# Lewis-Stuart-11/3DGS-to-PC

Measured on NVIDIA H100. Metric: Mpoints/sec (sample+colour) at 3M Gaussians/200 cams, 1/2/4/8 H100 vs CPU ref, higher is better.
Workload: dtype f32

## Files before the change

### 3dgs-to-pc_b200/csrc/colour_common.cuh

```cuda
#pragma once
#include "common.cuh"

#define QT_FLAG_DROPPED 1
#define QT_FLAG_BIG 2

#define NODE_NONE 0
#define NODE_EMPTY 1
#define NODE_SPLIT 2
#define NODE_LEAF 3

#define G2PC_RANGE_MAX_LEVEL 8
#define G2PC_RANGE_EMPTY 0x00000001u
__host__ __device__ __forceinline__ uint32_t g2pc_pack_range(int xlo, int xhi, int ylo, int yhi) {
    return (uint32_t)xlo | ((uint32_t)xhi << 8) | ((uint32_t)ylo << 16) | ((uint32_t)yhi << 24);
}
__host__ __device__ __forceinline__ void g2pc_unpack_range(uint32_t r, int& xlo, int& xhi, int& ylo, int& yhi) {
    xlo = (int)(r & 255u); xhi = (int)((r >> 8) & 255u); ylo = (int)((r >> 16) & 255u); yhi = (int)(r >> 24);
}

__device__ __forceinline__ bool g2pc_frame_skipped(const uint32_t* fail, int frame) {
    return (uint32_t)(frame + 1) >= *fail;
}

__device__ __forceinline__ bool g2pc_report_skipped_frame(const uint32_t* fail, int frame, int32_t* header) {
    if (!g2pc_frame_skipped(fail, frame)) return false;
    if (threadIdx.x == 0) { header[G2PC_HDR_POISON] = (int32_t)*fail; header[G2PC_HDR_FRAME] = frame; }
    return true;
}

__device__ __forceinline__ void g2pc_write_frame_header(int32_t* header, uint32_t* fail, int frame, int num_leaves,
                                                        long long inst_total, int total_pix, int need_deeper,
                                                        int leaf_over, int cap_over) {
    header[G2PC_HDR_NUM_LEAVES] = num_leaves;
    header[G2PC_HDR_TOTAL_INST] = (int32_t)(inst_total & 0xFFFFFFFFll);
    header[G2PC_HDR_TOTAL_INST_HI] = (int32_t)(inst_total >> 32);
    header[G2PC_HDR_TOTAL_PIX] = total_pix;
    header[G2PC_HDR_NEED_DEEPER] = need_deeper;
    header[G2PC_HDR_LEAF_OVERFLOW] = leaf_over;
    header[G2PC_HDR_CAP_OVERFLOW] = cap_over;
    header[G2PC_HDR_FRAME] = frame;
    if (need_deeper | leaf_over | cap_over) atomicMin(fail, (uint32_t)(frame + 1));
    const uint32_t f = *(volatile uint32_t*)fail;
    header[G2PC_HDR_POISON] = f == 0xFFFFFFFFu ? 0 : (int32_t)f;
}

template <int NT, int CAP, typename K, typename KeyF>
__device__ __forceinline__ void g2pc_launch_order(K* s_sort, int nl, KeyF key, K index_mask, int32_t* leaf_order) {
    if (nl > CAP) {
        for (int i = threadIdx.x; i < nl; i += NT) leaf_order[i] = i;
        return;
    }
    int m = 1;
    while (m < nl) m <<= 1;
    for (int i = threadIdx.x; i < m; i += NT) s_sort[i] = i < nl ? key(i) : ~(K)0;
    __syncthreads();
    for (int k = 2; k <= m; k <<= 1) {
        for (int j = k >> 1; j > 0; j >>= 1) {
            for (int i = threadIdx.x; i < m; i += NT) {
                const int ixj = i ^ j;
                if (ixj > i) {
                    const K a = s_sort[i], b = s_sort[ixj];
                    const bool up = (i & k) == 0;
                    if ((a > b) == up) { s_sort[i] = b; s_sort[ixj] = a; }
                }
            }
            __syncthreads();
        }
    }
    for (int i = threadIdx.x; i < nl; i += NT) leaf_order[i] = (int)(s_sort[i] & index_mask);
}

__device__ __forceinline__ float ex2_approx(float x) {
    float r;
    asm("ex2.approx.ftz.f32 %0, %1;" : "=f"(r) : "f"(x));
    return r;
}

__device__ __forceinline__ uint32_t smem_u32(const void* p) { return (uint32_t)__cvta_generic_to_shared(p); }

__device__ __forceinline__ void mbar_init(unsigned long long* bar, int count) {
    asm volatile("mbarrier.init.shared::cta.b64 [%0], %1;" ::"r"(smem_u32(bar)), "r"(count) : "memory");
}
__device__ __forceinline__ void mbar_wait(unsigned long long* bar, uint32_t parity) {
    asm volatile(
        "{\n"
        ".reg .pred p;\n"
        "WAIT_%=:\n"
        "mbarrier.try_wait.parity.shared::cta.b64 p, [%0], %1;\n"
        "@p bra DONE_%=;\n"
        "bra WAIT_%=;\n"
        "DONE_%=:\n"
        "}\n" ::"r"(smem_u32(bar)), "r"(parity) : "memory");
}
__device__ __forceinline__ void tma_load_1d(void* dst, const void* src, uint32_t bytes, unsigned long long* bar) {
    asm volatile("fence.proxy.async.shared::cta;" ::: "memory");
    asm volatile("mbarrier.arrive.expect_tx.shared::cta.b64 _, [%0], %1;" ::"r"(smem_u32(bar)), "r"(bytes) : "memory");
    asm volatile("cp.async.bulk.shared::cluster.global.mbarrier::complete_tx::bytes [%0], [%1], %2, [%3];" ::"r"(
                     smem_u32(dst)), "l"(src), "r"(bytes), "r"(smem_u32(bar)) : "memory");
}
__device__ __forceinline__ void cp_async16(void* dst, const void* src) {
    asm volatile("cp.async.cg.shared.global [%0], [%1], 16;" ::"r"(smem_u32(dst)), "l"(src) : "memory");
}
__device__ __forceinline__ void cp_async_commit() { asm volatile("cp.async.commit_group;" ::: "memory"); }
template <int N>
__device__ __forceinline__ void cp_async_wait() { asm volatile("cp.async.wait_group %0;" ::"n"(N) : "memory"); }

__device__ __forceinline__ void id_ring_init(unsigned long long* bar) {
    mbar_init(&bar[0], 1); mbar_init(&bar[1], 1); mbar_init(&bar[2], 1);
    asm volatile("fence.mbarrier_init.release.cluster;" ::: "memory");
}
template <int CH>
__device__ __forceinline__ void id_ring_issue(uint32_t (*ids)[CH], unsigned long long* bar, const uint32_t* list,
                                              int cnt, int c) {
    const int nl = min(CH, cnt - c * CH);
    tma_load_1d(&ids[c % 3][0], list + (int64_t)c * CH, (uint32_t)(((nl + 3) & ~3) * 4), &bar[c % 3]);
}
__device__ __forceinline__ void id_ring_wait(unsigned long long* bar, uint32_t& phase_bits, int c) {
    const int s = c % 3;
    mbar_wait(&bar[s], (phase_bits >> s) & 1u);
    phase_bits ^= 1u << s;
}

__device__ __forceinline__ int next_work_item(int32_t* counter, int* s_item) {
    if (threadIdx.x == 0) *s_item = atomicAdd(counter, 1);
    __syncthreads();
    const int item = *s_item;
    __syncthreads();
    return item;
}

template <typename Kernel>
int g2pc_resident_ctas(Kernel kernel, int threads, size_t smem, int fallback_per_sm) {
    int dev = 0, sms = 132, per_sm = fallback_per_sm;
    cudaGetDevice(&dev);
    cudaDeviceGetAttribute(&sms, cudaDevAttrMultiProcessorCount, dev);
    if (cudaOccupancyMaxActiveBlocksPerMultiprocessor(&per_sm, kernel, threads, smem) != cudaSuccess || per_sm < 1)
        per_sm = fallback_per_sm;
    return sms * per_sm;
}

template <typename Coef>
__device__ __forceinline__ float sh_channel(Coef s, int deg, float x, float y, float z) {
    const float C0 = 0.28209479177387814f, C1 = 0.4886025119029199f;
    const float C2[5] = {1.0925484305920792f, -1.0925484305920792f, 0.31539156525252005f, -1.0925484305920792f,
                         0.5462742152960396f};
    const float C3[7] = {-0.5900435899266435f, 2.890611442640554f, -0.4570457994644658f, 0.3731763325901154f,
                         -0.4570457994644658f, 1.445305721320277f, -0.5900435899266435f};
    const float xx = x * x, yy = y * y, zz = z * z, xy = x * y, yz = y * z, xz = x * z;
    float r = C0 * s(0);
    if (deg > 0) {
        r = r - C1 * y * s(1) + C1 * z * s(2) - C1 * x * s(3);
        if (deg > 1) {
            r = r + C2[0] * xy * s(4) + C2[1] * yz * s(5) + C2[2] * (2.0f * zz - xx - yy) * s(6) + C2[3] * xz * s(7) +
                C2[4] * (xx - yy) * s(8);
            if (deg > 2) {
                r = r + C3[0] * y * (3.0f * xx - yy) * s(9) + C3[1] * xy * z * s(10) +
                    C3[2] * y * (4.0f * zz - xx - yy) * s(11) + C3[3] * z * (2.0f * zz - 3.0f * xx - 3.0f * yy) * s(12) +
                    C3[4] * x * (4.0f * zz - xx - yy) * s(13) + C3[5] * z * (xx - yy) * s(14) +
                    C3[6] * x * (xx - 3.0f * yy) * s(15);
            }
        }
    }
    return fmaxf(r + 0.5f, 0.0f);
}

__host__ __device__ __forceinline__ int off2d(int l) { return ((1 << (2 * l)) - 1) / 3; }

struct QtMeta {
    int32_t num_levels;
    int32_t max_gaussians_per_tile;
    int32_t width, height;
};

struct QtTables {
    const int32_t* xs; const int32_t* xe; const int32_t* xf;
    const int32_t* ys; const int32_t* ye; const int32_t* yf;
};

inline QtTables make_tables(const int32_t* tables, int n1) {
    QtTables t;
    t.xs = tables; t.xe = tables + n1; t.xf = tables + 2 * n1;
    t.ys = tables + 3 * n1; t.ye = tables + 4 * n1; t.yf = tables + 5 * n1;
    return t;
}

__device__ __forceinline__ QtTables load_tables(const QtTables g, int n1, int32_t* smem) {
    for (int i = threadIdx.x; i < n1; i += blockDim.x) {
        smem[i] = g.xs[i];
        smem[n1 + i] = g.xe[i];
        smem[2 * n1 + i] = g.xf[i];
        smem[3 * n1 + i] = g.ys[i];
        smem[4 * n1 + i] = g.ye[i];
        smem[5 * n1 + i] = g.yf[i];
    }
    __syncthreads();
    QtTables s;
    s.xs = smem; s.xe = smem + n1; s.xf = smem + 2 * n1;
    s.ys = smem + 3 * n1; s.ye = smem + 4 * n1; s.yf = smem + 5 * n1;
    return s;
}

__device__ __forceinline__ void axis_range(const int32_t* __restrict__ s, const int32_t* __restrict__ e, int level,
                                           float rmin, float rmax, float inv_step, int& lo, int& hi) {
    const int n = 1 << level;
    if (!(rmax > rmin)) { lo = 1; hi = 0; return; }
    int a = min(n - 1, max(0, (int)(rmin * inv_step)));
    while (a < n && !((float)e[a] > rmin)) ++a;
    while (a > 0 && (float)e[a - 1] > rmin) --a;
    lo = a;
    a = min(n - 1, max(0, (int)(rmax * inv_step)));
    while (a >= 0 && !((float)s[a] < rmax)) --a;
    while (a + 1 < n && (float)s[a + 1] < rmax) ++a;
    hi = a;
}

__device__ __forceinline__ void axis_range_from(const int32_t* __restrict__ s, const int32_t* __restrict__ e, int level,
                                                float rmin, float rmax, int lo_guess, int hi_guess, int& lo, int& hi) {
    const int n = 1 << level;
    if (!(rmax > rmin)) { lo = 1; hi = 0; return; }
    int a = min(n - 1, max(0, lo_guess));
    while (a < n && !((float)e[a] > rmin)) ++a;
    while (a > 0 && (float)e[a - 1] > rmin) --a;
    lo = a;
    a = min(n - 1, max(0, hi_guess));
    while (a >= 0 && !((float)s[a] < rmax)) --a;
    while (a + 1 < n && (float)s[a + 1] < rmax) ++a;
    hi = a;
}

__device__ __forceinline__ bool axis_member(const int32_t* __restrict__ s, const int32_t* __restrict__ e,
                                            const int32_t* __restrict__ f, int i) {
    return !(f[i] & QT_FLAG_DROPPED) && e[i] > s[i];
}

constexpr int WARP_SMALL_AREA = 12;
template <typename F>
__device__ __forceinline__ void warp_for_each_node(uint32_t range, uint32_t payload, F f) {
    const int lane = threadIdx.x & 31;
    int xlo, xhi, ylo, yhi;
    g2pc_unpack_range(range, xlo, xhi, ylo, yhi);
    const int area = (xlo > xhi || ylo > yhi) ? 0 : (xhi - xlo + 1) * (yhi - ylo + 1);
    if (area > 0 && area <= WARP_SMALL_AREA)
        for (int iy = ylo; iy <= yhi; ++iy)
            for (int ix = xlo; ix <= xhi; ++ix) f(ix, iy, lane, payload);
    unsigned big = __ballot_sync(0xffffffffu, area > WARP_SMALL_AREA);
    while (big) {
        const int b = __ffs(big) - 1;
        big &= big - 1u;
        const uint32_t br = __shfl_sync(0xffffffffu, range, b);
        const uint32_t bp = __shfl_sync(0xffffffffu, payload, b);
        int bx, bxh, by, byh;
        g2pc_unpack_range(br, bx, bxh, by, byh);
        const int bw = bxh - bx + 1, bh = byh - by + 1;
        const int sh = bw <= 1 ? 0 : 32 - __clz(bw - 1);
        if (sh >= 5) {
            for (int ry = 0; ry < bh; ++ry)
                for (int rx = lane; rx < bw; rx += 32) f(bx + rx, by + ry, b, bp);
        } else {
            const int rx = lane & ((1 << sh) - 1);
            if (rx < bw)
                for (int ry = lane >> sh; ry < bh; ry += 32 >> sh) f(bx + rx, by + ry, b, bp);
        }
    }
}

__device__ __forceinline__ void gaussian_rect(float mx, float my, float radius, int W, int H, float& x0, float& x1,
                                              float& y0, float& y1) {
    const float wm = (float)W - 1.0f, hm = (float)H - 1.0f;
    x0 = fminf(fmaxf(mx - radius, 0.0f), wm);
    x1 = fminf(fmaxf(mx + radius, 0.0f), wm);
    y0 = fminf(fmaxf(my - radius, 0.0f), hm);
    y1 = fminf(fmaxf(my + radius, 0.0f), hm);
}
```

### 3dgs-to-pc_b200/csrc/core.cu

```cuda
#include <stdarg.h>
#include "common.cuh"

static thread_local char g_err[512] = "";

void g2pc_set_error(const char* fmt, ...) {
    va_list ap;
    va_start(ap, fmt);
    vsnprintf(g_err, sizeof(g_err), fmt, ap);
    va_end(ap);
}

extern "C" int g2pc_version(void) { return 110; }
extern "C" const char* g2pc_last_error(void) { return g_err; }
```

### 3dgs-to-pc_b200/csrc/s4_tree.cu

```cuda
#include <cub/cub.cuh>
#include "colour_common.cuh"

namespace {

constexpr int TB = 1024;
constexpr int SORT_CAP = 4096;

struct TreeParams {
    QtMeta meta;
    QtTables tab;
    int32_t n1;
    uint32_t* node_cnt;
    uint8_t* node_state;
    int32_t* node_leaf;
    g2pc_leaf_t* leaves;
    int32_t* leaf_order;
    int32_t max_leaves;
    int64_t inst_capacity, pix_capacity, matrix_capacity;
    int32_t ms_chunks;
    int32_t frame;
    int32_t* header;
    uint32_t* fail;
    int32_t* work_counters;
    int32_t nodes_2d;
};

__device__ __forceinline__ void deinterleave(int key, int level, int& ix, int& iy) {
    ix = 0; iy = 0;
    for (int b = 0; b < level; ++b) {
        iy |= ((key >> (2 * b)) & 1) << b;
        ix |= ((key >> (2 * b + 1)) & 1) << b;
    }
}

__global__ void __launch_bounds__(TB) tree_kernel(const TreeParams p) {
    __shared__ int s_warp[33];
    __shared__ int s_flags[2];
    __shared__ unsigned long long s_sort[SORT_CAP];
    if (g2pc_report_skipped_frame(p.fail, p.frame, p.header)) return;
    const int L = p.meta.num_levels;
    if (threadIdx.x == 0) { s_flags[0] = 0; s_flags[1] = 0; }
    __syncthreads();
    int leaf_base = 0;
    long long inst_total = 0;
    for (int l = 0; l < L; ++l) {
        const int nn = 1 << (2 * l);
        const int o1 = (1 << l) - 1, o2 = off2d(l);
        for (int k0 = 0; k0 < nn; k0 += TB) {
            const int key = k0 + threadIdx.x;
            int is_leaf = 0, node = -1, ix = 0, iy = 0;
            uint32_t cnt = 0;
            if (key < nn) {
                deinterleave(key, l, ix, iy);
                node = o2 + (iy << l) + ix;
                bool exists = (l == 0);
                if (l > 0) {
                    const int pnode = off2d(l - 1) + ((iy >> 1) << (l - 1)) + (ix >> 1);
                    exists = p.node_state[pnode] == NODE_SPLIT;
                }
                uint8_t st = NODE_NONE;
                int32_t nl = -1;
                if (exists) {
                    const int fx = p.tab.xf[o1 + ix], fy = p.tab.yf[o1 + iy];
                    if (!((fx | fy) & QT_FLAG_DROPPED)) {
                        cnt = p.node_cnt[node];
                        const bool big = ((fx | fy) & QT_FLAG_BIG) != 0;
                        if (cnt == 0) st = NODE_EMPTY;
                        else if (big || cnt > (uint32_t)p.meta.max_gaussians_per_tile) {
                            st = NODE_SPLIT;
                            nl = -2;
                            if (l == L - 1) { st = NODE_NONE; nl = -1; s_flags[0] = 1; }
                        } else {
                            st = NODE_LEAF;
                            is_leaf = 1;
                        }
                    }
                }
                p.node_state[node] = st;
                p.node_leaf[node] = nl;
            }
            int tot;
            const int pre = block_scan_1024(is_leaf, s_warp, tot);
            if (is_leaf) {
                const int li = leaf_base + pre;
                if (li < p.max_leaves) {
                    g2pc_leaf_t lf;
                    lf.r0 = p.tab.ys[o1 + iy];
                    lf.c0 = p.tab.xs[o1 + ix];
                    lf.w = p.tab.xe[o1 + ix] - lf.c0 + 1;
                    lf.h = p.tab.ye[o1 + iy] - lf.r0 + 1;
                    lf.inst_begin = 0;
                    lf.inst_count = (int32_t)cnt;
                    lf.pix_offset = 0;
                    lf.node = node;
                    p.leaves[li] = lf;
                    p.node_leaf[node] = li;
                } else {
                    s_flags[1] = 1;
                }
            }
            leaf_base += tot;
        }
        __syncthreads();
    }
    const int nl = leaf_base < p.max_leaves ? leaf_base : p.max_leaves;
    int pix_base = 0;
    for (int k0 = 0; k0 < nl; k0 += TB) {
        const int i = k0 + threadIdx.x;
        int c = 0, a = 0;
        if (i < nl) { c = (p.leaves[i].inst_count + 3) & ~3; a = p.leaves[i].w * p.leaves[i].h; }
        int tc, ta;
        const int pc = block_scan_1024(c, s_warp, tc);
        const int pa = block_scan_1024(a, s_warp, ta);
        if (i < nl) {
            p.leaves[i].inst_begin = (int32_t)(inst_total + pc);
            p.leaves[i].pix_offset = pix_base + pa;
        }
        inst_total += tc;
        pix_base += ta;
    }
    __syncthreads();
    g2pc_launch_order<TB, SORT_CAP>(s_sort, nl, [&](int i) {
        unsigned long long w = (unsigned long long)p.leaves[i].inst_count *
                               (unsigned long long)(p.leaves[i].w * p.leaves[i].h);
        w = w < (1ull << 44) - 1ull ? w : (1ull << 44) - 1ull;
        return (((1ull << 44) - 1ull - w) << 16) | (unsigned long long)i;
    }, 0xFFFFull, p.leaf_order);
    for (int k = threadIdx.x; k < p.nodes_2d; k += TB) p.node_cnt[k] = 0u;
    if (threadIdx.x < G2PC_WORK_COUNTERS) p.work_counters[threadIdx.x] = 0;
    if (threadIdx.x == 0) {
        const int cap_over = (inst_total > p.inst_capacity || (long long)pix_base > p.pix_capacity ||
                              (long long)p.ms_chunks * (long long)nl > p.matrix_capacity || inst_total > 0x7FFFFFFFll)
                                 ? 1 : 0;
        g2pc_write_frame_header(p.header, p.fail, p.frame, leaf_base, inst_total, pix_base, s_flags[0], s_flags[1],
                                cap_over);
    }
}

struct MsParams {
    const unsigned long long* val_sorted;
    int64_t n;
    const float4* proj;
    int32_t width, height;
    float inv_width, inv_height;
    QtMeta meta;
    QtTables tab;
    int32_t n1;
    uint32_t level_mask;
    int32_t base_level;
    const int32_t* node_leaf;
    const int32_t* header;
    const uint32_t* fail;
    int32_t frame;
    const g2pc_leaf_t* leaves;
    uint32_t* matrix;
    uint32_t* inst_gid;
    int32_t leaf_cap;
    int32_t base_clean;
    uint32_t clean_mask;
    int32_t grid_w;
    int32_t steps;
};

template <typename F>
__device__ __forceinline__ void for_each_leaf(const MsParams& p, const QtTables& T, const int32_t* __restrict__ s_leaf,
                                              uint32_t range, uint32_t gid, F f) {
    if (p.grid_w > 0) {
        warp_for_each_node(range, gid, [&](int ix, int iy, int owner, uint32_t og) { f(iy * p.grid_w + ix, owner, og); });
        return;
    }
    const int lb = p.base_level;
    const int o1 = (1 << lb) - 1;
    unsigned deeper = 0;
    if (p.base_clean) {
        warp_for_each_node(range, gid, [&](int ix, int iy, int owner, uint32_t og) {
            const int32_t v = s_leaf[(iy << lb) + ix];
            if (v >= 0) f(v, owner, og);
            else if (v == -2) deeper |= 1u << owner;
        });
    } else {
        warp_for_each_node(range, gid, [&](int ix, int iy, int owner, uint32_t og) {
            if (!axis_member(T.ys + o1, T.ye + o1, T.yf + o1, iy) || !axis_member(T.xs + o1, T.xe + o1, T.xf + o1, ix)) return;
            const int32_t v = s_leaf[(iy << lb) + ix];
            if (v >= 0) f(v, owner, og);
            else if (v == -2) deeper |= 1u << owner;
        });
    }
    if (p.meta.num_levels <= lb + 1) return;
    int xlo, xhi, ylo, yhi;
    g2pc_unpack_range(range, xlo, xhi, ylo, yhi);
#pragma unroll
    for (int o = 16; o > 0; o >>= 1) deeper |= __shfl_xor_sync(0xffffffffu, deeper, o);
    const int lane = threadIdx.x & 31;
    bool mine = (deeper >> lane) & 1u;
    if (!mine && xlo <= xhi) {
        const int ex = max(xlo - 1, 0), ey = max(ylo - 1, 0);
        for (int iy = ey; iy <= yhi; ++iy)
            for (int ix = ex; ix <= xhi; ++ix)
                if ((iy < ylo || ix < xlo) && s_leaf[(iy << lb) + ix] == -2) mine = true;
    }
    if (!__any_sync(0xffffffffu, mine)) return;
    float x0 = 0.f, x1 = 0.f, y0 = 0.f, y1 = 0.f;
    if (mine) {
        const float4 q0 = __ldg(p.proj + 3 * (int64_t)gid);
        const float4 q2 = __ldg(p.proj + 3 * (int64_t)gid + 2);
        gaussian_rect(q0.x, q0.y, q2.z, p.width, p.height, x0, x1, y0, y1);
    }
    const float isx0 = p.inv_width, isy0 = p.inv_height;
    for (int l = lb + 1; l < p.meta.num_levels; ++l) {
        if (!((p.level_mask >> l) & 1u)) continue;
        const int ol = (1 << l) - 1;
        int axlo = 1, axhi = 0, aylo = 1, ayhi = 0;
        if (mine) {
            axis_range(T.xs + ol, T.xe + ol, l, x0, x1, isx0 * (float)(1 << l), axlo, axhi);
            if (axlo <= axhi) axis_range(T.ys + ol, T.ye + ol, l, y0, y1, isy0 * (float)(1 << l), aylo, ayhi);
        }
        const bool some = axlo <= axhi && aylo <= ayhi;
        const int32_t* nl = p.node_leaf + off2d(l);
        if (((p.clean_mask >> l) & 1u) && l <= G2PC_RANGE_MAX_LEVEL) {
            const uint32_t rl = some ? g2pc_pack_range(axlo, axhi, aylo, ayhi) : (uint32_t)G2PC_RANGE_EMPTY;
            warp_for_each_node(rl, gid, [&](int ix, int iy, int owner, uint32_t og) {
                const int32_t v = __ldg(nl + (iy << l) + ix);
                if (v >= 0) f(v, owner, og);
            });
            continue;
        }
        if (!some) continue;
        for (int iy = aylo; iy <= ayhi; ++iy) {
            if (!axis_member(T.ys + ol, T.ye + ol, T.yf + ol, iy)) continue;
            for (int ix = axlo; ix <= axhi; ++ix) {
                if (!axis_member(T.xs + ol, T.xe + ol, T.xf + ol, ix)) continue;
                const int32_t v = __ldg(nl + (iy << l) + ix);
                if (v >= 0) f(v, lane, gid);
            }
        }
    }
}

__device__ __forceinline__ unsigned long long ms_entry(const MsParams& p, int64_t k) {
    return k < p.n ? p.val_sorted[k] : (unsigned long long)G2PC_RANGE_EMPTY << 32;
}

__device__ __forceinline__ int32_t* ms_load_common(const MsParams& p, int32_t* smem, QtTables& T) {
    if (p.grid_w > 0) { T = p.tab; return smem; }
    if (p.base_clean && p.meta.num_levels <= p.base_level + 1) {
        T = p.tab;
        __syncthreads();
    } else {
        T = load_tables(p.tab, p.n1, smem);
    }
    int32_t* s_leaf = smem + 6 * p.n1;
    const int nb = 1 << (2 * p.base_level);
    const int32_t* src = p.node_leaf + off2d(p.base_level);
    for (int i = threadIdx.x; i < nb; i += blockDim.x) s_leaf[i] = src[i];
    return s_leaf;
}

template <int C>
__global__ void __launch_bounds__(C, 1024 / C) ms_count_kernel(const MsParams p) {
    extern __shared__ int32_t smem_ms[];
    if (g2pc_frame_skipped(p.fail, p.frame)) return;
    const int nl = p.header[G2PC_HDR_NUM_LEAVES];
    QtTables T;
    int32_t* s_leaf = ms_load_common(p, smem_ms, T);
    uint32_t* s_hist = reinterpret_cast<uint32_t*>(s_leaf + (p.grid_w > 0 ? 0 : (1 << (2 * p.base_level))));
    for (int i = threadIdx.x; i < nl; i += C) s_hist[i] = 0u;
    __syncthreads();
    const int64_t k0 = (int64_t)blockIdx.x * p.steps * C;
    for (int s = 0; s < p.steps; ++s) {
        const int64_t b = k0 + (int64_t)s * C;
        if (b >= p.n) break;
        const unsigned long long v = ms_entry(p, b + threadIdx.x);
        for_each_leaf(p, T, s_leaf, (uint32_t)(v >> 32), (uint32_t)v,
                      [&](int leaf, int, uint32_t) { atomicAdd(s_hist + leaf, 1u); });
    }
    __syncthreads();
    uint32_t* row = p.matrix + (int64_t)blockIdx.x * nl;
    for (int i = threadIdx.x; i < nl; i += C) row[i] = s_hist[i];
}

constexpr int SCAN_BATCH = 8;
__global__ void __launch_bounds__(1024) ms_scan_kernel(const MsParams p, int32_t rows) {
    __shared__ uint32_t s_sum[32][33];
    if (g2pc_frame_skipped(p.fail, p.frame)) return;
    const int nl = p.header[G2PC_HDR_NUM_LEAVES];
    if (blockIdx.x * 32 >= nl) return;
    const int tx = threadIdx.x & 31, ty = threadIdx.x >> 5;
    const int leaf = blockIdx.x * 32 + tx;
    const int band = (rows + 31) / 32;
    const int r0 = min(rows, ty * band), r1 = min(rows, r0 + band);
    uint32_t* col = p.matrix + leaf;
    uint32_t sum = 0;
    if (leaf < nl) {
#pragma unroll 8
        for (int r = r0; r < r1; ++r) sum += col[(int64_t)r * nl];
    }
    s_sum[ty][tx] = sum;
    __syncthreads();
    if (leaf >= nl) return;
    uint32_t run = (uint32_t)p.leaves[leaf].inst_begin;
    for (int s = 0; s < ty; ++s) run += s_sum[s][tx];
    for (int r = r0; r < r1; r += SCAN_BATCH) {
        uint32_t c[SCAN_BATCH];
#pragma unroll
        for (int q = 0; q < SCAN_BATCH; ++q) c[q] = r + q < r1 ? col[(int64_t)(r + q) * nl] : 0u;
#pragma unroll
        for (int q = 0; q < SCAN_BATCH; ++q) {
            if (r + q < r1) col[(int64_t)(r + q) * nl] = run;
            run += c[q];
        }
    }
}

template <int C>
__global__ void __launch_bounds__(C, 768 / C) ms_scatter_kernel(const MsParams p) {
    extern __shared__ int32_t smem_ms[];
    if (g2pc_frame_skipped(p.fail, p.frame)) return;
    const int nl = p.header[G2PC_HDR_NUM_LEAVES];
    constexpr int WORDS = C / 32;
    QtTables T;
    int32_t* s_leaf = ms_load_common(p, smem_ms, T);
    uint32_t* s_row = reinterpret_cast<uint32_t*>(s_leaf + (p.grid_w > 0 ? 0 : (1 << (2 * p.base_level))));
    uint32_t* s_bits = s_row + p.leaf_cap;
    {
        const uint32_t* grow = p.matrix + (int64_t)blockIdx.x * nl;
        for (int i = threadIdx.x; i < nl; i += C) s_row[i] = grow[i];
        if (((reinterpret_cast<uintptr_t>(s_bits) & 15) == 0) && ((nl & 3) == 0)) {
            uint4* b4 = reinterpret_cast<uint4*>(s_bits);
            for (int i = threadIdx.x; i < WORDS * nl / 4; i += C) b4[i] = make_uint4(0u, 0u, 0u, 0u);
        } else {
            for (int i = threadIdx.x; i < WORDS * nl; i += C) s_bits[i] = 0u;
        }
    }
    __syncthreads();
    const int w = threadIdx.x >> 5;
    uint32_t* mybits = s_bits + w * nl;
    const int64_t k0 = (int64_t)blockIdx.x * p.steps * C;
    unsigned long long v = ms_entry(p, k0 + threadIdx.x);
    for (int s = 0; s < p.steps; ++s) {
        const int64_t b = k0 + (int64_t)s * C;
        if (b >= p.n) break;
        const bool more = s + 1 < p.steps && b + C < p.n;
        const uint32_t range = (uint32_t)(v >> 32), gid = (uint32_t)v;
        for_each_leaf(p, T, s_leaf, range, gid, [&](int leaf, int owner, uint32_t) { atomicOr(mybits + leaf, 1u << owner); });
        __syncthreads();
        const unsigned long long vn = more ? ms_entry(p, b + C + threadIdx.x) : 0ull;
        for_each_leaf(p, T, s_leaf, range, gid, [&](int leaf, int owner, uint32_t og) {
            uint32_t pos = s_row[leaf] + (uint32_t)__popc(mybits[leaf] & ((1u << owner) - 1u));
            for (int w2 = 0; w2 < w; ++w2) pos += (uint32_t)__popc(s_bits[w2 * nl + leaf]);
            p.inst_gid[pos] = og;
        });
        if (!more) break;
        __syncthreads();
        for (int i = threadIdx.x; i < nl; i += C) {
            uint32_t cnt = 0;
#pragma unroll
            for (int w2 = 0; w2 < WORDS; ++w2) {
                cnt += (uint32_t)__popc(s_bits[w2 * nl + i]);
                s_bits[w2 * nl + i] = 0u;
            }
            s_row[i] += cnt;
        }
        __syncthreads();
        v = vn;
    }
}

size_t align256(size_t x) { return (x + 255) & ~(size_t)255; }

constexpr int64_t MS_TARGET_CTAS = 4096;
constexpr int64_t MS_MAX_STEPS = 32;
int32_t ms_steps(int64_t n, int C) {
    const int64_t s = n / ((int64_t)C * MS_TARGET_CTAS);
    return (int32_t)(s < 1 ? 1 : (s > MS_MAX_STEPS ? MS_MAX_STEPS : s));
}

int32_t ms_chunks(int64_t n, int C) {
    const int64_t e = (int64_t)C * ms_steps(n, C);
    return (int32_t)((n + e - 1) / e);
}

template <int C>
int launch_multisplit(const MsParams& p, int32_t chunks, cudaStream_t st) {
    const size_t common = p.grid_w > 0 ? 0 : ((size_t)6 * p.n1 + ((size_t)1 << (2 * p.base_level))) * sizeof(int32_t);
    const size_t smem_count = common + (size_t)p.leaf_cap * sizeof(uint32_t);
    const size_t smem_scatter = common + (size_t)(C / 32 + 1) * p.leaf_cap * sizeof(uint32_t);
    if (smem_scatter > 200 * 1024 || smem_count > 200 * 1024) {
        g2pc_set_error("g2pc_multisplit: shared memory budget exceeded");
        return G2PC_ERR_INVALID;
    }
    if (smem_count > 48 * 1024)
        G2PC_CUDA(cudaFuncSetAttribute(ms_count_kernel<C>, cudaFuncAttributeMaxDynamicSharedMemorySize, (int)smem_count));
    if (smem_scatter > 48 * 1024)
        G2PC_CUDA(cudaFuncSetAttribute(ms_scatter_kernel<C>, cudaFuncAttributeMaxDynamicSharedMemorySize, (int)smem_scatter));
    ms_count_kernel<C><<<(unsigned)chunks, C, smem_count, st>>>(p);
    G2PC_CHECK_LAUNCH();
    ms_scan_kernel<<<(unsigned)((p.leaf_cap + 31) / 32), 1024, 0, st>>>(p, chunks);
    G2PC_CHECK_LAUNCH();
    ms_scatter_kernel<C><<<(unsigned)chunks, C, smem_scatter, st>>>(p);
    G2PC_CHECK_LAUNCH();
    return G2PC_OK;
}

int run_multisplit(MsParams p, int C, cudaStream_t st) {
    p.steps = ms_steps(p.n, C);
    const int32_t chunks = ms_chunks(p.n, C);
    if (C == 256) return launch_multisplit<256>(p, chunks, st);
    if (C == 128) return launch_multisplit<128>(p, chunks, st);
    return launch_multisplit<64>(p, chunks, st);
}

}

extern "C" int g2pc_build_tree(const int32_t* tables, int32_t num_levels, int32_t max_gaussians_per_tile,
                               uint32_t* node_cnt, uint8_t* node_state, int32_t* node_leaf, g2pc_leaf_t* leaves,
                               int32_t* leaf_order, int32_t max_leaves, int64_t inst_capacity, int64_t pix_capacity,
                               int64_t matrix_capacity, int32_t ms_chunks, int32_t frame, int32_t* header,
                               uint32_t* fail, int32_t* work_counters, void* stream) {
    G2PC_CHECK_ARG(tables && node_cnt && node_state && node_leaf && leaves && leaf_order && header && fail &&
                       work_counters, "null pointer");
    G2PC_CHECK_ARG(num_levels >= 1 && num_levels <= G2PC_MAX_LEVELS && max_leaves >= 1, "bad sizes");
    G2PC_CHECK_ARG(frame >= 0 && ms_chunks >= 0, "bad frame / chunk count");
    TreeParams p;
    p.meta.num_levels = num_levels; p.meta.max_gaussians_per_tile = max_gaussians_per_tile;
    p.meta.width = 0; p.meta.height = 0;
    p.n1 = (1 << num_levels) - 1;
    p.tab = make_tables(tables, p.n1);
    p.node_cnt = node_cnt; p.node_state = node_state; p.node_leaf = node_leaf; p.leaves = leaves;
    p.leaf_order = leaf_order; p.max_leaves = max_leaves;
    p.inst_capacity = inst_capacity; p.pix_capacity = pix_capacity; p.matrix_capacity = matrix_capacity;
    p.ms_chunks = ms_chunks; p.frame = frame; p.header = header; p.fail = fail; p.work_counters = work_counters;
    p.nodes_2d = off2d(num_levels);
    tree_kernel<<<1, TB, 0, (cudaStream_t)stream>>>(p);
    G2PC_CHECK_LAUNCH();
    return G2PC_OK;
}

extern "C" int64_t g2pc_depth_sort_workspace_bytes(int64_t n) {
    size_t sort_b = 0;
    cub::DeviceRadixSort::SortPairs(nullptr, sort_b, (const uint32_t*)nullptr, (uint32_t*)nullptr,
                                    (const unsigned long long*)nullptr, (unsigned long long*)nullptr, n);
    return (int64_t)(align256((size_t)n * 4) + align256(sort_b));
}

extern "C" int g2pc_depth_sort(const uint32_t* depth_key, const uint64_t* val, int64_t n, uint64_t* val_sorted,
                               void* workspace, int64_t workspace_bytes, void* stream) {
    G2PC_CHECK_ARG(n >= 0, "n < 0");
    if (n == 0) return G2PC_OK;
    G2PC_CHECK_ARG(depth_key && val && val_sorted && workspace, "null pointer");
    G2PC_CHECK_ARG(workspace_bytes >= g2pc_depth_sort_workspace_bytes(n), "workspace too small");
    char* ws = (char*)workspace;
    uint32_t* keys_out = (uint32_t*)ws;
    void* tmp = ws + align256((size_t)n * 4);
    size_t b = (size_t)workspace_bytes - align256((size_t)n * 4);
    G2PC_CUDA(cub::DeviceRadixSort::SortPairs(tmp, b, depth_key, keys_out, (const unsigned long long*)val,
                                              (unsigned long long*)val_sorted, n, 0, 32, (cudaStream_t)stream));
    return G2PC_OK;
}

extern "C" int32_t g2pc_multisplit_chunk(int32_t leaf_cap) {
    const int64_t n = leaf_cap;
    if (n * 36 <= 74 * 1024) return 256;
    if (n * 20 <= 74 * 1024) return 128;
    if (n * 12 <= 110 * 1024) return 64;
    if (n * 20 <= 200 * 1024) return 128;
    if (n * 12 <= 200 * 1024) return 64;
    return 0;
}

extern "C" int32_t g2pc_multisplit_rows(int64_t n, int32_t leaf_cap) {
    const int C = g2pc_multisplit_chunk(leaf_cap);
    if (C <= 0) return 0;
    return ms_chunks(n, C);
}

extern "C" int g2pc_multisplit(const uint64_t* val_sorted, int64_t n, const void* proj, int32_t width, int32_t height,
                               const int32_t* tables, int32_t num_levels, uint32_t level_mask, uint32_t clean_mask,
                               const int32_t* node_leaf,
                               const g2pc_leaf_t* leaves, const int32_t* header, const uint32_t* fail, int32_t frame,
                               int32_t leaf_cap, uint32_t* matrix, uint32_t* inst_gid, void* stream) {
    G2PC_CHECK_ARG(n >= 0, "n < 0");
    if (n == 0) return G2PC_OK;
    G2PC_CHECK_ARG(val_sorted && proj && tables && node_leaf && leaves && header && fail && matrix && inst_gid,
                   "null pointer");
    G2PC_CHECK_ARG(num_levels >= 1 && num_levels <= G2PC_MAX_LEVELS && level_mask != 0u, "bad levels");
    const int C = g2pc_multisplit_chunk(leaf_cap);
    G2PC_CHECK_ARG(C > 0, "too many leaves for the multisplit");
    MsParams p;
    p.val_sorted = (const unsigned long long*)val_sorted; p.n = n; p.proj = (const float4*)proj;
    p.width = width; p.height = height;
    p.inv_width = 1.0f / (float)width; p.inv_height = 1.0f / (float)height;
    p.meta.num_levels = num_levels; p.meta.max_gaussians_per_tile = 0; p.meta.width = width; p.meta.height = height;
    p.n1 = (1 << num_levels) - 1;
    p.tab = make_tables(tables, p.n1);
    p.level_mask = level_mask; p.base_level = __builtin_ctz(level_mask);
    G2PC_CHECK_ARG(p.base_level <= G2PC_RANGE_MAX_LEVEL, "first leaf-candidate level too deep");
    p.node_leaf = node_leaf; p.header = header; p.fail = fail; p.frame = frame; p.leaves = leaves; p.matrix = matrix;
    p.inst_gid = inst_gid;
    p.leaf_cap = leaf_cap; p.grid_w = 0;
    p.base_clean = (int32_t)((clean_mask >> p.base_level) & 1u);
    p.clean_mask = clean_mask;
    return run_multisplit(p, C, (cudaStream_t)stream);
}

extern "C" int g2pc_multisplit_grid(const uint64_t* val_sorted, int64_t n, int32_t grid_w, int32_t grid_h,
                                    const g2pc_leaf_t* leaves, const int32_t* header, const uint32_t* fail,
                                    int32_t frame, int32_t leaf_cap, uint32_t* matrix, uint32_t* inst_gid, void* stream) {
    G2PC_CHECK_ARG(n >= 0, "n < 0");
    if (n == 0) return G2PC_OK;
    G2PC_CHECK_ARG(val_sorted && leaves && header && fail && matrix && inst_gid, "null pointer");
    G2PC_CHECK_ARG(grid_w >= 1 && grid_h >= 1 && grid_w <= 256 && grid_h <= 256 && leaf_cap >= grid_w * grid_h,
                   "bad tile grid / leaf_cap");
    const int C = g2pc_multisplit_chunk(leaf_cap);
    G2PC_CHECK_ARG(C > 0, "too many tiles for the multisplit");
    MsParams p{};
    p.val_sorted = (const unsigned long long*)val_sorted; p.n = n;
    p.meta.num_levels = 1;
    p.level_mask = 1u;
    p.header = header; p.fail = fail; p.frame = frame; p.leaves = leaves; p.matrix = matrix;
    p.inst_gid = inst_gid;
    p.leaf_cap = leaf_cap; p.grid_w = grid_w; p.base_clean = 1; p.clean_mask = 1u;
    return run_multisplit(p, C, (cudaStream_t)stream);
}
```

### 3dgs-to-pc_b200/g2pc/capi.py

```python
import contextlib
import ctypes
import os

import torch

HERE = os.path.dirname(os.path.abspath(__file__))
LIB_PATH = os.path.join(HERE, "libg2pc.so")

F32, F64 = 0, 1
CULL_EPS_NORM, CULL_EXPLICIT = 0, 1
ST_OVERFLOW, ST_CHOLFAIL, ST_CHOLREG, ST_WORDS = 0, 1, 2, 4

_c_void_p = ctypes.c_void_p
_i32, _i64, _u32, _u64, _f32 = ctypes.c_int32, ctypes.c_int64, ctypes.c_uint32, ctypes.c_uint64, ctypes.c_float

SIGNATURES = {
    "g2pc_version": ([], ctypes.c_int),
    "g2pc_last_error": ([], ctypes.c_char_p),
    "g2pc_cov_build": ([_c_void_p, _c_void_p, ctypes.c_int, _f32, _i64, _c_void_p, _c_void_p], ctypes.c_int),
    "g2pc_normals": ([_c_void_p, _c_void_p, ctypes.c_int, _i64, _c_void_p, _c_void_p], ctypes.c_int),
    "g2pc_eigvals_sym3": ([_c_void_p, _i64, _c_void_p, _c_void_p], ctypes.c_int),
    "g2pc_sample_count": ([_c_void_p, _c_void_p, _c_void_p, ctypes.c_int, _c_void_p, _c_void_p, _c_void_p, _i64, _i64,
                           _c_void_p, _i32, _i32, _i32, _f32, _i32, _u64, _u32, _c_void_p, _c_void_p, _c_void_p,
                           _c_void_p, _c_void_p], ctypes.c_int),
    "g2pc_sample_emit_chunk_points": ([], ctypes.c_int),
    "g2pc_sample_emit": ([_c_void_p, _c_void_p, _i64, _c_void_p, _c_void_p, _c_void_p, _i32, _u64, _u32, _c_void_p,
                          _c_void_p, _c_void_p, ctypes.c_int, _i64, _c_void_p], ctypes.c_int),
    "g2pc_dump_eps": ([_c_void_p, _i64, _i32, _i32, _u64, _u32, _c_void_p, _c_void_p], ctypes.c_int),
    "g2pc_cull_workspace_bytes": ([_i64], ctypes.c_int64),
    "g2pc_cull_select": ([_c_void_p, _f32, _c_void_p, _f32, _c_void_p, _c_void_p, _c_void_p, _c_void_p, _c_void_p,
                          _c_void_p, _i64, _i64, _i64, _c_void_p, _c_void_p, _c_void_p, _i64, _c_void_p], ctypes.c_int),
    "g2pc_gather_rows": ([_c_void_p, _i64, _i32, _c_void_p, _c_void_p, _c_void_p, _c_void_p], ctypes.c_int),
    "g2pc_ppg_workspace_bytes": ([_i64], ctypes.c_int64),
    "g2pc_knn_workspace_bytes": ([_i64], ctypes.c_int64),
    "g2pc_knn_mean_dist": ([_c_void_p, _i64, _i32, _c_void_p, _c_void_p, _c_void_p, _i64, _c_void_p], ctypes.c_int),
    "g2pc_knn_ids": ([_c_void_p, _i64, _i32, _c_void_p, _c_void_p, _c_void_p, _c_void_p, _i64, _c_void_p], ctypes.c_int),
    "g2pc_sor_workspace_bytes": ([_i64], ctypes.c_int64),
    "g2pc_sor_mask": ([_c_void_p, _i64, ctypes.c_double, _c_void_p, _c_void_p, _c_void_p, _i64, _c_void_p], ctypes.c_int),
    "g2pc_mesh_splat_workspace_bytes": ([_i64], ctypes.c_int64),
    "g2pc_mesh_splat": ([_c_void_p, _c_void_p, ctypes.c_int, _i64, _i32, _c_void_p, _c_void_p, _c_void_p, _c_void_p,
                         _c_void_p, _i64, _c_void_p], ctypes.c_int),
    "g2pc_mesh_solve_workspace_bytes": ([_i32], ctypes.c_int64),
    "g2pc_mesh_vcycle": ([_c_void_p, _c_void_p, _i32, _c_void_p, _i32, _c_void_p, _c_void_p, _i64, _c_void_p],
                         ctypes.c_int),
    "g2pc_mesh_iso_workspace_bytes": ([], ctypes.c_int64),
    "g2pc_mesh_iso": ([_c_void_p, _c_void_p, _i64, _c_void_p, _i32, _c_void_p, _c_void_p, _c_void_p, _i64, _c_void_p],
                      ctypes.c_int),
    "g2pc_mesh_extract_workspace_bytes": ([_i32], ctypes.c_int64),
    "g2pc_mesh_extract_count": ([_c_void_p, _i32, _c_void_p, _c_void_p, _c_void_p, _i64, _c_void_p], ctypes.c_int),
    "g2pc_mesh_extract_emit": ([_c_void_p, _i32, _c_void_p, _c_void_p, _c_void_p, _i64, _c_void_p, _i64, _c_void_p,
                                _c_void_p, _c_void_p, _c_void_p, _c_void_p], ctypes.c_int),
    "g2pc_mesh_gather_workspace_bytes": ([_i64], ctypes.c_int64),
    "g2pc_mesh_gather": ([_c_void_p, _c_void_p, _c_void_p, _i64, _c_void_p, _i32, _c_void_p, _c_void_p, _i64, _c_void_p,
                          _i64, _c_void_p, _c_void_p, _c_void_p, _i64, _c_void_p], ctypes.c_int),
    "g2pc_mesh_trim_workspace_bytes": ([_i64, _i64], ctypes.c_int64),
    "g2pc_mesh_trim": ([_c_void_p, _c_void_p, _c_void_p, _i64, _c_void_p, _i64, _c_void_p, _c_void_p, _c_void_p,
                        _c_void_p, _c_void_p, _c_void_p, _c_void_p, _c_void_p, _i64, _c_void_p], ctypes.c_int),
    "g2pc_mesh_smooth_workspace_bytes": ([_i64, _i64], ctypes.c_int64),
    "g2pc_mesh_smooth": ([_c_void_p, _i64, _c_void_p, _i64, _i32, _c_void_p, _i64, _c_void_p], ctypes.c_int),
    "g2pc_mesh_normals_workspace_bytes": ([_i64, _i64], ctypes.c_int64),
    "g2pc_mesh_normals": ([_c_void_p, _i64, _c_void_p, _i64, _c_void_p, _c_void_p, _c_void_p, _i64, _c_void_p],
                          ctypes.c_int),
    "g2pc_mesh_band_bricks_workspace_bytes": ([_i32], ctypes.c_int64),
    "g2pc_mesh_band_bricks": ([_c_void_p, _c_void_p, _i64, _c_void_p, _i32, _c_void_p, _c_void_p, _c_void_p, _c_void_p,
                               _c_void_p, _i64, _c_void_p], ctypes.c_int),
    "g2pc_mesh_band_list": ([_c_void_p, _i32, _c_void_p, _c_void_p], ctypes.c_int),
    "g2pc_mesh_band_splat": ([_c_void_p, _c_void_p, ctypes.c_int, _c_void_p, _i64, _c_void_p, _i32, _c_void_p, _i64,
                              _c_void_p, _c_void_p, _c_void_p], ctypes.c_int),
    "g2pc_mesh_band_ghosts": ([_c_void_p, _c_void_p, _i32, _c_void_p, _c_void_p, _i64, _c_void_p, _c_void_p, _c_void_p,
                               _c_void_p, _c_void_p, _c_void_p], ctypes.c_int),
    "g2pc_mesh_band_cg_workspace_bytes": ([_i64], ctypes.c_int64),
    "g2pc_mesh_band_cg_start": ([_c_void_p, _i32, _c_void_p, _c_void_p, _i64, _c_void_p, _c_void_p, _c_void_p, _i64,
                                 _c_void_p], ctypes.c_int),
    "g2pc_mesh_band_cg_step": ([_c_void_p, _i32, _c_void_p, _c_void_p, _i64, _c_void_p, _i32, _c_void_p, _c_void_p,
                                _i64, _c_void_p], ctypes.c_int),
    "g2pc_mesh_band_iso_workspace_bytes": ([], ctypes.c_int64),
    "g2pc_mesh_band_iso": ([_c_void_p, _c_void_p, _i64, _c_void_p, _i32, _c_void_p, _c_void_p, _c_void_p, _c_void_p,
                            _i64, _c_void_p], ctypes.c_int),
    "g2pc_mesh_band_extract_workspace_bytes": ([_i64], ctypes.c_int64),
    "g2pc_mesh_band_extract_count": ([_c_void_p, _i32, _c_void_p, _c_void_p, _i64, _c_void_p, _c_void_p, _c_void_p,
                                      _i64, _c_void_p], ctypes.c_int),
    "g2pc_mesh_band_extract_emit": ([_c_void_p, _i32, _c_void_p, _c_void_p, _i64, _c_void_p, _c_void_p, _c_void_p, _i64,
                                     _c_void_p, _i64, _c_void_p, _c_void_p, _c_void_p, _c_void_p, _c_void_p],
                                    ctypes.c_int),
    "g2pc_mesh_band_gather_workspace_bytes": ([_i64], ctypes.c_int64),
    "g2pc_mesh_band_gather": ([_c_void_p, _c_void_p, _c_void_p, _i64, _c_void_p, _i32, _c_void_p, _c_void_p, _i64,
                               _c_void_p, _c_void_p, _c_void_p, _i64, _c_void_p], ctypes.c_int),
    "g2pc_mesh_decimate_prepare_workspace_bytes": ([_i64, _i64], ctypes.c_int64),
    "g2pc_mesh_decimate_prepare": ([_c_void_p, _i64, _c_void_p, _i64, _c_void_p, _c_void_p, _c_void_p, _i64, _c_void_p],
                                   ctypes.c_int),
    "g2pc_mesh_decimate_round_workspace_bytes": ([_i64, _i64], ctypes.c_int64),
    "g2pc_mesh_decimate_select": ([_c_void_p, _i64, _c_void_p, _i64, _c_void_p, _c_void_p, _c_void_p, _c_void_p, _i64,
                                   _c_void_p], ctypes.c_int),
    "g2pc_mesh_decimate_apply": ([_c_void_p, _i64, _c_void_p, _i64, _c_void_p, _c_void_p, _c_void_p, _c_void_p,
                                  _c_void_p, _i64, _i64, _c_void_p, _c_void_p, _c_void_p, _c_void_p, _c_void_p, _i64,
                                  _c_void_p], ctypes.c_int),
    "g2pc_mesh_decimate_finish_workspace_bytes": ([_i64], ctypes.c_int64),
    "g2pc_mesh_decimate_finish": ([_c_void_p, _i64, _c_void_p, _i64, _c_void_p, _c_void_p, _c_void_p, _c_void_p,
                                   _c_void_p, _c_void_p, _c_void_p, _c_void_p, _c_void_p, _c_void_p, _i64, _c_void_p],
                                  ctypes.c_int),
    "g2pc_tsdf_frame_workspace_bytes": ([_i64], ctypes.c_int64),
    "g2pc_tsdf_frame": ([_c_void_p, _i64, _i32, _c_void_p, _c_void_p, _i64, _c_void_p], ctypes.c_int),
    "g2pc_tsdf_integrate": ([_c_void_p, _i32, ctypes.c_double, _c_void_p, _c_void_p, _c_void_p, _c_void_p, _i32, _i32,
                             _c_void_p, _c_void_p, _c_void_p, _i32, _c_void_p, _c_void_p, _c_void_p, _c_void_p],
                            ctypes.c_int),
    "g2pc_tsdf_compact_workspace_bytes": ([_i64, _i64], ctypes.c_int64),
    "g2pc_tsdf_gather_compact": ([_c_void_p, _c_void_p, _i32, _c_void_p, _c_void_p, _c_void_p, _i64, _c_void_p, _i64,
                                  _c_void_p, _c_void_p, _c_void_p, _c_void_p, _c_void_p, _c_void_p, _c_void_p,
                                  _c_void_p, _c_void_p, _i64, _c_void_p], ctypes.c_int),
    "g2pc_orient_prepare_workspace_bytes": ([_i64], ctypes.c_int64),
    "g2pc_orient_prepare": ([_c_void_p, _c_void_p, ctypes.c_int, _i64, _c_void_p, _c_void_p, _c_void_p, _c_void_p,
                             _c_void_p, _i64, _c_void_p], ctypes.c_int),
    "g2pc_orient_edges_workspace_bytes": ([_i64, _i32], ctypes.c_int64),
    "g2pc_orient_edges": ([_c_void_p, _i64, _i32, _c_void_p, _c_void_p, _c_void_p, _c_void_p, _c_void_p, _c_void_p,
                           _i64, _c_void_p], ctypes.c_int),
    "g2pc_orient_round_workspace_bytes": ([_i64, _i64], ctypes.c_int64),
    "g2pc_orient_round": ([_c_void_p, _c_void_p, _c_void_p, _i64, _i64, _i32, _i64, _c_void_p, _c_void_p, _c_void_p,
                           _c_void_p, _c_void_p, _i64, _c_void_p], ctypes.c_int),
    "g2pc_orient_finish_workspace_bytes": ([_i64], ctypes.c_int64),
    "g2pc_orient_finish": ([_c_void_p, _c_void_p, _c_void_p, _i64, _c_void_p, ctypes.c_int, _i64, _c_void_p, _c_void_p,
                            _c_void_p, _c_void_p, _c_void_p, _c_void_p, _c_void_p, _i64, _c_void_p], ctypes.c_int),
    "g2pc_face_cameras": ([_c_void_p, _c_void_p, ctypes.c_int, _c_void_p, _i64, _c_void_p, _i64, _c_void_p, _i64,
                           _c_void_p, _c_void_p, _c_void_p], ctypes.c_int),
    "g2pc_points_per_gaussian": ([_c_void_p, _c_void_p, _i64, ctypes.c_double, _c_void_p, _c_void_p, _c_void_p, _i64,
                                  _c_void_p], ctypes.c_int),
    "g2pc_pack_geometry": ([_c_void_p, _c_void_p, _c_void_p, _i64, _c_void_p, _c_void_p], ctypes.c_int),
    "g2pc_preprocess": ([_c_void_p, _c_void_p, _c_void_p, _i32, _i32, _i64, _c_void_p, _c_void_p, _c_void_p, _i32, _u32,
                         _u32, _c_void_p, _c_void_p, _c_void_p, _c_void_p, _c_void_p], ctypes.c_int),
    "g2pc_preprocess_cameras": ([_c_void_p, _c_void_p, _c_void_p, _i32, _i32, _i64, _c_void_p, _i32, _c_void_p,
                                 _c_void_p, _i32, _u32, _u32, _c_void_p, _c_void_p, _c_void_p, _c_void_p, _c_void_p],
                                ctypes.c_int),
    "g2pc_depth_sort_workspace_bytes": ([_i64], ctypes.c_int64),
    "g2pc_depth_sort": ([_c_void_p, _c_void_p, _i64, _c_void_p, _c_void_p, _i64, _c_void_p], ctypes.c_int),
    "g2pc_build_tree": ([_c_void_p, _i32, _i32, _c_void_p, _c_void_p, _c_void_p, _c_void_p, _c_void_p, _i32, _i64, _i64,
                         _i64, _i32, _i32, _c_void_p, _c_void_p, _c_void_p, _c_void_p], ctypes.c_int),
    "g2pc_multisplit_chunk": ([_i32], ctypes.c_int32),
    "g2pc_multisplit_rows": ([_i64, _i32], ctypes.c_int32),
    "g2pc_multisplit": ([_c_void_p, _i64, _c_void_p, _i32, _i32, _c_void_p, _i32, _u32, _u32, _c_void_p, _c_void_p,
                         _c_void_p, _c_void_p, _i32, _i32, _c_void_p, _c_void_p, _c_void_p], ctypes.c_int),
    "g2pc_blend": ([_c_void_p, _c_void_p, _c_void_p, _c_void_p, _i32, _i32, _i32, _c_void_p, _c_void_p, _c_void_p,
                    _c_void_p, _c_void_p, _c_void_p, _i32, _i32, _f32, _f32, _c_void_p, _c_void_p, _c_void_p],
                   ctypes.c_int),
    "g2pc_blend_set_compact": ([ctypes.c_int], None),
    "g2pc_blend_set_cull": ([ctypes.c_int], None),
    "g2pc_accumulate": ([_c_void_p, _c_void_p, _i64, _c_void_p, _c_void_p, _c_void_p, _i32, _c_void_p], ctypes.c_int),
    "g2pc_tiles_preprocess": ([_c_void_p, _c_void_p, _c_void_p, _i32, _i32, _i32, _i64, _c_void_p, _c_void_p, _c_void_p,
                               _c_void_p, _c_void_p, _c_void_p, _c_void_p], ctypes.c_int),
    "g2pc_tiles_build": ([_c_void_p, _i32, _i32, _c_void_p, _c_void_p, _i32, _i64, _i64, _i32, _i32, _c_void_p,
                          _c_void_p, _c_void_p, _c_void_p], ctypes.c_int),
    "g2pc_multisplit_grid": ([_c_void_p, _i64, _i32, _i32, _c_void_p, _c_void_p, _c_void_p, _i32, _i32, _c_void_p,
                              _c_void_p, _c_void_p], ctypes.c_int),
    "g2pc_tiles_blend": ([_c_void_p, _c_void_p, _c_void_p, _c_void_p, _i32, _c_void_p, _c_void_p, _c_void_p, _c_void_p,
                          _c_void_p, _c_void_p, _c_void_p, _c_void_p, _i32, _i32, _c_void_p, _c_void_p, _c_void_p,
                          _c_void_p], ctypes.c_int),
    "g2pc_tiles_blend_fusion": ([_c_void_p, _c_void_p, _c_void_p, _c_void_p, _i32, _c_void_p, _c_void_p, _c_void_p,
                                 _c_void_p, _c_void_p, _c_void_p, _c_void_p, _c_void_p, _i32, _i32, _c_void_p, _c_void_p,
                                 _c_void_p, _c_void_p, _c_void_p, _c_void_p], ctypes.c_int),
    "g2pc_tiles_accumulate": ([_c_void_p, _c_void_p, _c_void_p, _i32, _i32, _i64, _c_void_p, _c_void_p, _c_void_p,
                               _c_void_p, _c_void_p, _i32, _c_void_p, _c_void_p, _c_void_p, _c_void_p], ctypes.c_int),
    "g2pc_fill_u32": ([_c_void_p, _u32, _i64, _c_void_p], ctypes.c_int),
    "g2pc_compose_image": ([_c_void_p, _c_void_p, _i32, _i32, _f32, _c_void_p, _c_void_p], ctypes.c_int),
}


class Raster(ctypes.Structure):
    _fields_ = [("viewmatrix", _f32 * 16), ("projmatrix", _f32 * 16), ("campos", _f32 * 3), ("tan_fovx", _f32),
                ("tan_fovy", _f32), ("width", _i32), ("height", _i32)]


class Camera(ctypes.Structure):
    _fields_ = [("view", _f32 * 16), ("proj", _f32 * 16), ("campos", _f32 * 3), ("tan_fovx", _f32),
                ("tan_fovy", _f32), ("focal_x", _f32), ("focal_y", _f32), ("width", _i32), ("height", _i32)]


(HDR_NUM_LEAVES, HDR_TOTAL_INST, HDR_TOTAL_PIX, HDR_NEED_DEEPER, HDR_LEAF_OVERFLOW, HDR_CAP_OVERFLOW, HDR_POISON,
 HDR_FRAME, HDR_TOTAL_INST_HI) = range(9)
HDR_WORDS = 16
WORK_COUNTERS = 4
STAT_WARP_GAUSSIANS, STAT_WORDS = 0, 4
LEAF_WORDS = 8
PREPROCESS_MAX_CAMERAS = 8

_lib = None


class G2pcError(RuntimeError):
    pass


def load(path=None):
    global _lib
    if _lib is not None and path is None:
        return _lib
    path = path or LIB_PATH
    if not os.path.exists(path):
        raise G2pcError(
            f"{path} not found: build it with `python -m g2pc.build` (or __graft_entry__.build()). "
            "There is no CPU fallback for the g2pc kernels.")
    lib = ctypes.CDLL(path)
    for name, (argtypes, restype) in SIGNATURES.items():
        fn = getattr(lib, name)
        fn.argtypes = argtypes
        fn.restype = restype
    _lib = lib
    return lib


LAUNCHES = 0
TIMING = None
_OWN_KERNELS = {"g2pc_multisplit": 3, "g2pc_multisplit_grid": 3, "g2pc_depth_sort": 0, "g2pc_cull_select": 3,
                "g2pc_points_per_gaussian": 5, "g2pc_knn_mean_dist": 6, "g2pc_knn_ids": 6, "g2pc_sor_mask": 5, "g2pc_mesh_splat": 5,
                "g2pc_mesh_iso": 7, "g2pc_mesh_extract_count": 2, "g2pc_mesh_extract_emit": 2, "g2pc_mesh_gather": 3,
                "g2pc_mesh_trim": 6, "g2pc_mesh_normals": 3, "g2pc_mesh_band_bricks": 4, "g2pc_mesh_band_cg_start": 4,
                "g2pc_mesh_band_cg_step": 6,
                "g2pc_mesh_band_iso": 4, "g2pc_mesh_band_extract_count": 2, "g2pc_mesh_band_extract_emit": 2,
                "g2pc_mesh_band_gather": 2, "g2pc_mesh_decimate_prepare": 4, "g2pc_mesh_decimate_select": 8,
                "g2pc_mesh_decimate_apply": 5, "g2pc_mesh_decimate_finish": 4, "g2pc_orient_prepare": 2, "g2pc_orient_edges": 2,
                "g2pc_orient_round": 5, "g2pc_orient_finish": 3, "g2pc_tsdf_frame": 2, "g2pc_tsdf_gather_compact": 4}
_NOT_KERNELS = {"g2pc_version", "g2pc_last_error", "g2pc_sample_emit_chunk_points", "g2pc_multisplit_chunk",
                "g2pc_multisplit_rows", "g2pc_blend_set_compact", "g2pc_blend_set_cull"}


def call(name, *args):
    global LAUNCHES
    fn = getattr(load(), name)
    if TIMING is None or name in _NOT_KERNELS or name.endswith("_workspace_bytes"):
        status = fn(*args)
    else:
        with phase(TIMING, name):
            status = fn(*args)
    LAUNCHES += _OWN_KERNELS.get(name, 1)
    check(status, name)


@contextlib.contextmanager
def phase(timings, name):
    if timings is None:
        yield
        return
    a, b = torch.cuda.Event(enable_timing=True), torch.cuda.Event(enable_timing=True)
    a.record()
    yield
    b.record()
    timings.setdefault(name, []).append((a, b))


def check(status, what):
    if status != 0:
        msg = load().g2pc_last_error()
        raise G2pcError(f"{what} failed (status {status}): {msg.decode() if msg else ''}")


def ptr(t):
    if t is None:
        return None
    return t.data_ptr()


def workspace(nbytes, device):
    return torch.empty((max(int(nbytes), 256),), dtype=torch.uint8, device=device)


def stream_ptr(device=None):
    return torch.cuda.current_stream(device).cuda_stream


def dtype_code(t):
    if t.dtype == torch.float32:
        return F32
    if t.dtype == torch.float64:
        return F64
    raise G2pcError(f"unsupported dtype {t.dtype} (need float32 or float64)")


def require_cuda(*tensors):
    for t in tensors:
        if t is not None and not t.is_cuda:
            raise G2pcError("g2pc kernels need CUDA tensors; there is no CPU fallback "
                            f"(got a tensor on {t.device})")


def check_cloud(points, normals=None, colours=None, what=None):
    if what is not None and normals is None:
        raise G2pcError(f"{what} needs normals (the cloud has none)")
    if points is None:
        raise G2pcError(f"{what or 'the point-cloud kernels'} needs the points")
    require_cuda(points, normals, colours)
    if points.dim() != 2 or points.shape[1] != 3 or points.dtype != torch.float32:
        raise G2pcError(f"points must be (n, 3) float32, got {tuple(points.shape)} {points.dtype}")
    if normals is not None and (normals.shape != points.shape or normals.dtype not in (torch.float32, torch.float64)):
        raise G2pcError(f"normals must be (n, 3) float32 or float64 like the points, got {tuple(normals.shape)} "
                        f"{normals.dtype}")
    if colours is not None and colours.shape != points.shape:
        raise G2pcError(f"colours must be (n, 3) like the points, got {tuple(colours.shape)}")
    devices = [str(t.device) for t in (points, normals, colours) if t is not None]
    if len(set(devices)) > 1:
        raise G2pcError(f"the points, normals and colours are on different devices ({', '.join(devices)})")


def gather_rows(index, m, tensors):
    dev = index.device
    srcs = [t.contiguous() for t in tensors]
    dsts = [torch.empty((m,) + tuple(s.shape[1:]), dtype=s.dtype, device=dev) for s in srcs]
    if m > 0:
        k = len(srcs)
        call("g2pc_gather_rows", ptr(index), m, k, (ctypes.c_void_p * k)(*[s.data_ptr() for s in srcs]),
             (ctypes.c_void_p * k)(*[d.data_ptr() for d in dsts]),
             (ctypes.c_int32 * k)(*[s[0].numel() * s.element_size() for s in srcs]), stream_ptr(dev))
    return dsts
```

### 3dgs-to-pc_b200/g2pc/frames.py

```python
import torch

from . import capi, config


_HDR_POOLS = {}


def _resolution(camera):
    return int(camera.image_width), int(camera.image_height)


def total_instances(h):
    return h[capi.HDR_TOTAL_INST] + (h[capi.HDR_TOTAL_INST_HI] << 32)


class FrameQueue:

    def _init_frames(self, preprocess_cameras=1):
        self._frame = 0
        self._pending = []
        self._deferred = []
        self._batch = 0
        self.preprocess_cameras = preprocess_cameras
        self._hdr_pool = _HDR_POOLS.setdefault(str(self.device), [])
        self.replays = 0
        self.async_mode = False
        self.num_slots = max(1, int(config.FRAME_SLOTS))
        self._streams = [torch.cuda.Stream(device=self.device) for _ in range(self.num_slots)]
        self._fail = torch.full((1,), -1, dtype=torch.int32, device=self.device)
        self._prev_done = None
        dev, m = self.device, max(self._n, 1)
        nbytes = int(self.lib.g2pc_depth_sort_workspace_bytes(m))
        self._slots = [dict(proj=torch.empty((m, 12), dtype=torch.float32, device=dev),
                            depth_key=torch.empty((m,), dtype=torch.int32, device=dev),
                            val=torch.empty((m,), dtype=torch.int64, device=dev),
                            val_sorted=torch.empty((m,), dtype=torch.int64, device=dev),
                            depth_ws=torch.empty((max(nbytes, 1),), dtype=torch.uint8, device=dev),
                            hdr=torch.zeros((capi.HDR_WORDS,), dtype=torch.int32, device=dev),
                            work=torch.zeros((capi.WORK_COUNTERS,), dtype=torch.int32, device=dev),
                            inst_gid=None, matrix=None) for _ in range(self.num_slots)]
        self._pre_sets = [[sl] + [None] * (preprocess_cameras - 1) for sl in self._slots]
        self._set_free = [None] * self.num_slots
        self._pre_stream = torch.cuda.Stream(device=self.device) if preprocess_cameras > 1 else None
        self._cam_best = torch.zeros((m,), dtype=torch.int64, device=dev)
        self._stats = torch.zeros((capi.STAT_WORDS,), dtype=torch.int64, device=dev)
        self._inst_cap = max(8 * self._n, 1 << 16)
        self._tables = {}
        self._last_slot = 0
        self.last_stats = {}

    def _grow_lists(self, sl, leaf_cap, rows):
        need = self._inst_cap + 4 * leaf_cap + 64
        if sl["inst_gid"] is None or sl["inst_gid"].numel() < need:
            sl["inst_gid"] = torch.empty((need,), dtype=torch.int32, device=self.device)
        mneed = rows * leaf_cap
        if sl["matrix"] is None or sl["matrix"].numel() < mneed:
            sl["matrix"] = torch.empty((max(mneed, 1),), dtype=torch.int32, device=self.device)

    def _depth_sort(self, sl, stream, pre=None):
        pre = sl if pre is None else pre
        capi.call("g2pc_depth_sort", capi.ptr(pre["depth_key"]), capi.ptr(pre["val"]), self._n, capi.ptr(sl["val_sorted"]),
                  capi.ptr(sl["depth_ws"]), sl["depth_ws"].numel(), stream)

    def _grow_inst_cap(self, h):
        total = total_instances(h)
        if total > 0x7FFFFFFF:
            raise capi.G2pcError(f"{total} (Gaussian, tile) instances in one camera: more than 2^31 - 1")
        self._inst_cap = max(self._inst_cap, int(1.25 * total) + 1024)

    def _reset_counts(self):
        for t in self._tables.values():
            for ts in t["slots"]:
                ts["node_cnt"].zero_()
            for cnts in t.get("pre_cnt", []):
                for c in cnts:
                    c.zero_()

    def executed_pairs(self):
        self.flush()
        return int(self._stats[capi.STAT_WARP_GAUSSIANS].item()) * 128

    def get_gaussian_colours(self):
        self.flush()
        return self.gaussian_colours * 255

    def _pre_set(self, bset, j):
        sets = self._pre_sets[bset]
        if sets[j] is None:
            m = max(self._n, 1)
            sets[j] = dict(proj=torch.empty((m, 12), dtype=torch.float32, device=self.device),
                           depth_key=torch.empty((m,), dtype=torch.int32, device=self.device),
                           val=torch.empty((m,), dtype=torch.int64, device=self.device))
        return sets[j]

    def _enqueue_preprocess(self, cameras, bset):
        """Owners whose front half projects each camera itself (the CUDA back-end) have nothing to do here."""

    def _launch_batch(self, batch):
        bset = self._batch % self.num_slots
        self._batch += 1
        for j, (frame, camera, _) in enumerate(batch):
            self._ensure_buffers(camera, frame % self.num_slots)
            self._pre_set(bset, j)
        ready = torch.cuda.Event()
        ready.record(torch.cuda.current_stream(self.device))
        st0 = self._pre_stream if self._pre_stream is not None else self._streams[batch[0][0] % self.num_slots]
        st0.wait_event(ready)
        if self._set_free[bset] is not None:
            st0.wait_event(self._set_free[bset])
        with torch.cuda.stream(st0):
            self._enqueue_preprocess([camera for _, camera, _ in batch], bset)
        projected = torch.cuda.Event()
        projected.record(st0)
        for j, (frame, camera, camera_index) in enumerate(batch):
            slot = frame % self.num_slots
            st = self._streams[slot]
            if st is not st0:
                st.wait_event(projected)
            with torch.cuda.stream(st):
                dev_hdr = self._enqueue_front(camera, frame, slot, (bset, j))
                hdr = self._hdr_pool.pop() if self._hdr_pool else torch.zeros((capi.HDR_WORDS,), dtype=torch.int32).pin_memory()
                hdr.copy_(dev_hdr, non_blocking=True)
                if self._prev_done is not None:
                    st.wait_event(self._prev_done)
                self._enqueue_back(camera, frame, camera_index, slot)
                done = torch.cuda.Event()
                done.record(st)
            self._prev_done = done
            self._pending.append((frame, camera, camera_index, hdr, done))
        self._set_free[bset] = self._prev_done

    def _launch_frames(self, frames):
        batch = []
        for item in frames:
            if batch and (len(batch) == self.preprocess_cameras or _resolution(batch[0][1]) != _resolution(item[1])):
                self._launch_batch(batch)
                batch = []
            batch.append(item)
        if batch:
            self._launch_batch(batch)

    def _submit(self, camera, camera_index=None):
        frame = self._frame
        self._frame += 1
        camera_index = frame if camera_index is None else camera_index
        self._deferred.append((frame, camera, camera_index))
        if not self.async_mode:
            self.flush()
        else:
            if len(self._deferred) >= self.preprocess_cameras:
                self._launch_deferred()
            self._poll(block_if_more_than=8)

    def _launch_deferred(self):
        frames, self._deferred = self._deferred, []
        self._launch_frames(frames)

    def _poll(self, block_if_more_than=None):
        while self._pending:
            frame, camera, cidx, hdr, ev = self._pending[0]
            if not ev.query():
                if block_if_more_than is None or len(self._pending) <= block_if_more_than:
                    return
                ev.synchronize()
            h = hdr.tolist()
            if h[capi.HDR_POISON] and h[capi.HDR_POISON] - 1 <= frame:
                self._recover(h)
                continue
            self._confirm(h)
            self._hdr_pool.append(hdr)
            self._pending.pop(0)

    def flush(self):
        self._launch_deferred()
        while self._pending:
            self._pending[-1][4].synchronize()
            self._poll(block_if_more_than=0)
        if self._prev_done is not None:
            torch.cuda.current_stream(self.device).wait_event(self._prev_done)

    def _all_streams(self):
        return self._streams + ([self._pre_stream] if self._pre_stream is not None else [])

    def _recover(self, h):
        for st in self._all_streams():
            st.synchronize()
        failed = h[capi.HDR_POISON] - 1
        todo = [p for p in self._pending if p[0] >= failed]
        self._pending = [p for p in self._pending if p[0] < failed]
        self._fix(h)
        self._fail.fill_(-1)
        self._reset_counts()
        torch.cuda.current_stream(self.device).synchronize()
        self.replays += 1
        for (frame, camera, cidx, hdr, ev) in todo:
            self._hdr_pool.append(hdr)
        self._launch_frames([(frame, camera, cidx) for (frame, camera, cidx, hdr, ev) in todo])

    def __del__(self):
        try:
            for st in self._all_streams():
                st.synchronize()
        except Exception:
            pass
```

### 3dgs-to-pc_b200/g2pc/rasterizer.py

```python
import ctypes
import math
from typing import NamedTuple

import torch

from . import capi
from .frames import FrameQueue, total_instances

FLT_MAX_BITS = 0x7F7FFFFF
TILE = 16


class GaussianRasterizationSettings(NamedTuple):
    image_height: int
    image_width: int
    tanfovx: float
    tanfovy: float
    bg: torch.Tensor
    scale_modifier: float
    viewmatrix: torch.Tensor
    projmatrix: torch.Tensor
    sh_degree: int
    campos: torch.Tensor
    mask: torch.Tensor
    prefiltered: bool
    debug: bool
    antialiasing: bool


def _host_list(t, n):
    if isinstance(t, (list, tuple)):
        v = [float(x) for x in t]
    else:
        v = t.detach().to("cpu", torch.float32).reshape(-1).tolist()
    if len(v) != n:
        raise ValueError(f"expected {n} values, got {len(v)}")
    return v


def _raster_struct(rs):
    c = capi.Raster()
    V = getattr(rs, "_viewmatrix_host", None) or _host_list(rs.viewmatrix, 16)
    P = getattr(rs, "_projmatrix_host", None) or _host_list(rs.projmatrix, 16)
    pos = getattr(rs, "_campos_host", None) or _host_list(rs.campos, 3)
    for i in range(16):
        c.viewmatrix[i] = V[i]
        c.projmatrix[i] = P[i]
    for i in range(3):
        c.campos[i] = pos[i]
    c.tan_fovx, c.tan_fovy = float(rs.tanfovx), float(rs.tanfovy)
    c.width, c.height = int(rs.image_width), int(rs.image_height)
    return c


def _cov6_to_full(cov6):
    c = cov6.to(torch.float32)
    return torch.stack([c[:, 0], c[:, 1], c[:, 2], c[:, 1], c[:, 3], c[:, 4], c[:, 2], c[:, 4], c[:, 5]], 1).reshape(-1, 3, 3)


def _cov_from_scale_rot(scales, rotations, mod):
    q = rotations.to(torch.float32)
    r, x, y, z = q[:, 0], q[:, 1], q[:, 2], q[:, 3]
    R = torch.stack([1 - 2 * (y * y + z * z), 2 * (x * y - r * z), 2 * (x * z + r * y),
                     2 * (x * y + r * z), 1 - 2 * (x * x + z * z), 2 * (y * z - r * x),
                     2 * (x * z - r * y), 2 * (y * z + r * x), 1 - 2 * (x * x + y * y)], 1).reshape(-1, 3, 3)
    L = R * (mod * scales.to(torch.float32))[:, None, :]
    return L @ L.transpose(1, 2)


class GaussianRasterizer(FrameQueue):

    def __init__(self, means3D, means2D, opacities, shs=None, colors_precomp=None, scales=None, rotations=None,
                 cov3D_precomp=None, visible_gaussian_threshold=0.0, surface_distance_std=None,
                 calculate_surface_distance=False, sh_layout=0):
        if (shs is None and colors_precomp is None) or (shs is not None and colors_precomp is not None):
            raise Exception('Please provide excatly one of either SHs or precomputed colors!')
        if ((scales is None or rotations is None) and cov3D_precomp is None) or \
                ((scales is not None or rotations is not None) and cov3D_precomp is not None):
            raise Exception('Please provide exactly one of either scale/rotation pair or precomputed 3D covariance!')
        capi.require_cuda(means3D, opacities, shs, colors_precomp, scales, rotations, cov3D_precomp)
        self.lib = capi.load()
        self.means3D = means3D.to(torch.float32).contiguous()
        self.means2D = means2D
        self.opacities = opacities
        self.shs = shs if shs is not None else torch.Tensor([])
        self.colors_precomp = colors_precomp if colors_precomp is not None else torch.Tensor([])
        self.scales = scales if scales is not None else torch.Tensor([])
        self.rotations = rotations if rotations is not None else torch.Tensor([])
        self.cov3D_precomp = cov3D_precomp if cov3D_precomp is not None else torch.Tensor([])
        self.device = self.means3D.device
        dev = self.device
        n = self.means3D.shape[0]
        self._n = n

        self.gaussian_max_contribution = torch.zeros(n, device=dev, dtype=torch.float)
        self.gaussian_min_surface_distance = torch.full((n,), torch.finfo(torch.float).max, device=dev, dtype=torch.float)
        self.gaussian_total_contribution = torch.zeros(n, device=dev, dtype=torch.float)
        self.gaussian_colours = torch.zeros((n, 3), device=dev, dtype=torch.float)
        self.visible_gaussian_threshold = visible_gaussian_threshold
        self.surface_distance_std = surface_distance_std
        self.calculate_surface_distance = calculate_surface_distance
        self.first_frame = None

        self._scale_modifier = None
        self._geom = torch.empty((max(n, 1), 12), dtype=torch.float32, device=dev)
        self._packed = False
        self._colour_f32 = colors_precomp.to(torch.float32).contiguous() if colors_precomp is not None else None
        self._shs_f32 = None
        self._sh_layout = int(sh_layout)
        if shs is not None:
            self._shs_f32 = shs.to(torch.float32).contiguous()
            self._sh_stride = int(self._shs_f32.shape[2] if self._sh_layout == 0 else self._shs_f32.shape[1])
        self._init_frames()
        m = max(n, 1)
        for sl in self._slots:
            sl["radii"] = torch.zeros((m,), dtype=torch.int32, device=dev)
        self._cam_dist = None
        if calculate_surface_distance:
            self._cam_dist = torch.empty((m,), dtype=torch.int32, device=dev)
            capi.call("g2pc_fill_u32", capi.ptr(self._cam_dist), FLT_MAX_BITS, m, capi.stream_ptr(dev))

    def __call__(self, raster_settings, **kw):
        return self.forward(raster_settings, **kw)

    def _pack(self, scale_modifier):
        if self._packed and self._scale_modifier == scale_modifier:
            return
        if self.cov3D_precomp.numel():
            cov = _cov6_to_full(self.cov3D_precomp) if self.cov3D_precomp.dim() == 2 else self.cov3D_precomp.to(torch.float32)
        else:
            cov = _cov_from_scale_rot(self.scales, self.rotations, float(scale_modifier))
        op = self.opacities.to(torch.float32).reshape(-1).contiguous()
        capi.call("g2pc_pack_geometry", capi.ptr(self.means3D), capi.ptr(cov.contiguous()), capi.ptr(op), self._n,
                  capi.ptr(self._geom), capi.stream_ptr(self.device))
        self._packed, self._scale_modifier = True, scale_modifier

    def _res_tables(self, W, H):
        t = self._tables.get((W, H))
        if t is None:
            dev = self.device
            gx, gy = ((W + TILE - 1) // TILE + 1) // 2, ((H + TILE - 1) // TILE + 1) // 2
            ntiles = gx * gy
            chunk = int(self.lib.g2pc_multisplit_chunk(ntiles))
            if chunk <= 0:
                raise capi.G2pcError(f"{ntiles} tiles: image too large for the multisplit tables")
            t = dict(gx=gx, gy=gy, ntiles=ntiles, rows=int(self.lib.g2pc_multisplit_rows(self._n, ntiles)),
                     slots=[dict(node_cnt=torch.zeros((ntiles,), dtype=torch.int32, device=dev),
                                 leaves=torch.zeros((ntiles, capi.LEAF_WORDS), dtype=torch.int32, device=dev),
                                 leaf_order=torch.zeros((ntiles,), dtype=torch.int32, device=dev))
                            for _ in range(self.num_slots)],
                     colour=torch.zeros((3, H, W), dtype=torch.float32, device=dev),
                     depth=torch.zeros((1, H, W), dtype=torch.float32, device=dev),
                     invdepth=torch.zeros((1, H, W), dtype=torch.float32, device=dev))
            self._tables[(W, H)] = t
        return t

    def _mask_of(self, rs, W, H):
        mask = rs.mask
        if mask is None:
            return None
        if not mask.is_cuda:
            raise capi.G2pcError("mask must be a CUDA tensor")
        if mask.numel() != W * H:
            raise capi.G2pcError("mask must have image_height * image_width entries")
        return mask.to(torch.int32).contiguous()

    def _ensure_buffers(self, rs, slot):
        self._pack(float(rs.scale_modifier))
        t = self._res_tables(int(rs.image_width), int(rs.image_height))
        self._grow_lists(self._slots[slot], t["ntiles"], t["rows"])
        self._slots[slot]["mask"] = self._mask_of(rs, int(rs.image_width), int(rs.image_height))

    def _enqueue_front(self, rs, frame, slot, pre=None):
        st = capi.stream_ptr(self.device)
        W, H = int(rs.image_width), int(rs.image_height)
        n = self._n
        t = self._res_tables(W, H)
        sl, ts = self._slots[slot], t["slots"][slot]
        c = _raster_struct(rs)
        deg = int(rs.sh_degree) if self._shs_f32 is not None else 0
        capi.call("g2pc_tiles_preprocess", capi.ptr(self._geom), capi.ptr(self._colour_f32), capi.ptr(self._shs_f32),
                  self._sh_stride if self._shs_f32 is not None else 0, min(deg, 3), self._sh_layout, n, ctypes.byref(c),
                  capi.ptr(sl["proj"]), capi.ptr(ts["node_cnt"]), capi.ptr(sl["depth_key"]), capi.ptr(sl["val"]),
                  capi.ptr(sl["radii"]), st)
        self._depth_sort(sl, st)
        capi.call("g2pc_tiles_build", capi.ptr(ts["node_cnt"]), W, H, capi.ptr(ts["leaves"]), capi.ptr(ts["leaf_order"]),
                  t["ntiles"], self._inst_cap, sl["matrix"].numel(), t["rows"], frame, capi.ptr(sl["hdr"]),
                  capi.ptr(self._fail), capi.ptr(sl["work"]), st)
        capi.call("g2pc_multisplit_grid", capi.ptr(sl["val_sorted"]), n, t["gx"], t["gy"], capi.ptr(ts["leaves"]),
                  capi.ptr(sl["hdr"]), capi.ptr(self._fail), frame, t["ntiles"], capi.ptr(sl["matrix"]),
                  capi.ptr(sl["inst_gid"]), st)
        self._last, self._last_slot = t, slot
        return sl["hdr"]

    def _enqueue_back(self, rs, frame, camera_index, slot):
        st = capi.stream_ptr(self.device)
        W, H = int(rs.image_width), int(rs.image_height)
        n = self._n
        t = self._res_tables(W, H)
        sl, ts = self._slots[slot], t["slots"][slot]
        mask = sl.get("mask")
        if mask is not None:
            t["colour"].zero_(); t["depth"].zero_(); t["invdepth"].zero_()
        bg = (ctypes.c_float * 3)(*(getattr(rs, "_bg_host", None) or _host_list(rs.bg, 3)))
        capi.call("g2pc_tiles_blend", capi.ptr(ts["leaves"]), capi.ptr(ts["leaf_order"]), capi.ptr(sl["hdr"]),
                  capi.ptr(self._fail), frame, capi.ptr(sl["inst_gid"]), capi.ptr(sl["proj"]), capi.ptr(self._cam_best),
                  capi.ptr(self._cam_dist), capi.ptr(mask), capi.ptr(t["colour"]), capi.ptr(t["depth"]),
                  capi.ptr(t["invdepth"]), W, H, bg, capi.ptr(sl["work"]), capi.ptr(self._stats), st)
        pc = getattr(self, "_per_camera", None) or (None, None, None)
        capi.call("g2pc_tiles_accumulate", capi.ptr(self._cam_best), capi.ptr(self._cam_dist), capi.ptr(t["colour"]), W, H,
                  n, capi.ptr(self.gaussian_max_contribution), capi.ptr(self.gaussian_total_contribution),
                  capi.ptr(self.gaussian_colours), capi.ptr(self.gaussian_min_surface_distance),
                  capi.ptr(self.first_frame), int(camera_index), capi.ptr(pc[0]), capi.ptr(pc[1]), capi.ptr(pc[2]), st)

    def forward(self, raster_settings, camera_index=None):
        self._submit(raster_settings, camera_index)
        t, radii = self._last, self._slots[self._last_slot]["radii"]
        if self.async_mode:
            return t["colour"], radii, t["invdepth"], t["depth"]
        return t["colour"].clone(), radii.clone(), t["invdepth"].clone(), t["depth"].clone()

    def _confirm(self, h):
        self.last_stats = dict(num_tiles=h[capi.HDR_NUM_LEAVES], frame=h[capi.HDR_FRAME],
                               total_instances=total_instances(h))

    def _fix(self, h):
        if not h[capi.HDR_CAP_OVERFLOW]:
            raise capi.G2pcError("failed frame header without a recoverable cause")
        self._grow_inst_cap(h)

    def update_max_contributions(self, new_gauss_contributions, new_gauss_colours):
        self.flush()
        upd = new_gauss_contributions > self.gaussian_max_contribution
        self.gaussian_max_contribution[upd] = new_gauss_contributions[upd]
        self.gaussian_colours[upd] = new_gauss_colours[upd]
        self.gaussian_total_contribution += new_gauss_contributions

    def update_min_surface_distances(self, new_gauss_surface_distances):
        self.flush()
        upd = new_gauss_surface_distances < self.gaussian_min_surface_distance
        self.gaussian_min_surface_distance[upd] = new_gauss_surface_distances[upd]

    def get_max_gaussian_contributions(self):
        self.flush()
        return self.gaussian_max_contribution

    def get_total_gaussian_contributions(self):
        self.flush()
        return self.gaussian_total_contribution

    def get_gaussians_above_contribution_threshold(self, contribution_threshold):
        return self.get_max_gaussian_contributions() > contribution_threshold

    def get_gaussians_above_total_contribution_threshold(self, contribution_threshold):
        return self.get_total_gaussian_contributions() > contribution_threshold

    def get_surface_gaussians_below_distance_threshold(self, surface_distance_threshold):
        if not self.calculate_surface_distance:
            raise Exception("Cannot determine Gaussian surface distance as this feature was not set at the start of rendering")
        self.flush()
        finite = self.gaussian_min_surface_distance < torch.finfo(torch.float).max
        mean_and_std = torch.std_mean(self.gaussian_min_surface_distance[finite])
        return self.gaussian_min_surface_distance < mean_and_std[1] * surface_distance_threshold

    def get_visible_gaussians(self):
        return self.get_gaussians_above_contribution_threshold(self.visible_gaussian_threshold)

    def get_gaussians_with_low_surface_distance(self):
        return self.get_surface_gaussians_below_distance_threshold(self.surface_distance_std)

    def get_predicted_surface_gaussians(self, predicted_surface_std=0.5):
        return self.get_surface_gaussians_below_distance_threshold(predicted_surface_std)


def rasterize_gaussians(background, means3D, colors, opacity, scales, rotations, scale_modifier, cov3D_precomp,
                        viewmatrix, projmatrix, tan_fovx, tan_fovy, image_height, image_width, sh, degree, campos, mask,
                        prefiltered, antialiasing, calculate_surface_distance, debug):
    if antialiasing:
        raise NotImplementedError("antialiasing=True is not part of the path (camera_handler.py:107 always passes False)")
    has_sh = sh is not None and sh.numel() > 0
    R = GaussianRasterizer(means3D, None, opacity, shs=sh if has_sh else None,
                           colors_precomp=None if has_sh else colors,
                           scales=scales if (cov3D_precomp is None or cov3D_precomp.numel() == 0) else None,
                           rotations=rotations if (cov3D_precomp is None or cov3D_precomp.numel() == 0) else None,
                           cov3D_precomp=cov3D_precomp if (cov3D_precomp is not None and cov3D_precomp.numel()) else None,
                           calculate_surface_distance=bool(calculate_surface_distance), sh_layout=1)
    n = means3D.shape[0]
    dev = means3D.device
    rs = GaussianRasterizationSettings(image_height=int(image_height), image_width=int(image_width), tanfovx=tan_fovx,
                                       tanfovy=tan_fovy, bg=background, scale_modifier=scale_modifier,
                                       viewmatrix=viewmatrix, projmatrix=projmatrix, sh_degree=int(degree), campos=campos,
                                       mask=mask, prefiltered=prefiltered, debug=debug, antialiasing=False)
    contrib = torch.zeros((n,), dtype=torch.float32, device=dev)
    pixels = torch.zeros((n,), dtype=torch.int32, device=dev)
    surf = torch.full((n,), torch.finfo(torch.float).max, dtype=torch.float32, device=dev)
    R._per_camera = (contrib, pixels, surf if calculate_surface_distance else None)
    R._submit(rs)
    R.flush()
    t = R._last
    empty = torch.empty((0,), dtype=torch.uint8, device=dev)
    return (int(R.last_stats["total_instances"]), t["colour"], t["depth"], R._slots[R._last_slot]["radii"], empty,
            empty.clone(), empty.clone(), t["invdepth"], contrib, surf, pixels)


def mark_visible(means3D, viewmatrix, projmatrix):
    V = viewmatrix.to(torch.float32)
    z = means3D.to(torch.float32) @ V[:3, 2] + V[3, 2]
    return z > 0.2
```

### 3dgs-to-pc_b200/gauss_render.py

```python
import ctypes
import math

import numpy as np
import torch

from g2pc import capi, config, quadtree
from g2pc.frames import FrameQueue, total_instances

C0 = 0.28209479177387814
C1 = 0.4886025119029199

homogeneous = lambda points: torch.cat([points, torch.ones_like(points[..., :1])], dim=-1)


def strip_lowerdiag(L):
    idx = torch.tensor([0, 1, 2, 4, 5, 8], device=L.device)
    return L.reshape(L.shape[0], 9).index_select(1, idx).to(torch.float)


def strip_symmetric(sym):
    return strip_lowerdiag(sym)


class GaussPythonRenderer(FrameQueue):

    def __init__(self, means3D, opacity, colour, cov3d, white_bkgd=True, visible_gaussian_threshold=0.0, shs=None,
                 sh_degree=None):
        capi.require_cuda(means3D, opacity, colour, cov3d, shs)
        self.lib = capi.load()
        self.white_bkgd = white_bkgd
        self.device = means3D.device
        n = means3D.shape[0]
        dev = self.device

        self.gaussian_max_contribution = torch.zeros(n, device=dev, dtype=torch.float32)
        self.gaussian_total_contribution = torch.zeros(n, device=dev, dtype=torch.float32)
        self.gaussian_colours = torch.zeros((n, 3), device=dev, dtype=torch.float32)
        self.visible_gaussian_threshold = visible_gaussian_threshold

        self.means3D = means3D.to(torch.float32).contiguous()
        self.opacity = opacity.to(torch.float32).reshape(-1).contiguous()
        self.cov3d = cov3d.to(torch.float32).contiguous()
        self.colour = colour
        self._colour_f32 = None if colour is None else colour.to(torch.float32).contiguous()
        self.shs = None
        self.sh_degree = 0
        if shs is not None:
            self.shs = shs.to(torch.float32).contiguous()
            ncoef = self.shs.shape[-1]
            deg = int(round(math.sqrt(ncoef))) - 1 if sh_degree is None else int(sh_degree)
            self.sh_degree = min(deg, 3)

        self.max_tile_size = config.MAX_TILE_SIZE
        self.max_gaussians_per_tile = config.MAX_GAUSSIANS_PER_TILE
        self.t_stop = config.BLEND_T_STOP
        self.compose_image = True
        self.async_mode = False
        self.first_frame = None
        self._extra_levels = 0
        self._n = n
        st = capi.stream_ptr(dev)
        self._geom = torch.empty((max(n, 1), 12), dtype=torch.float32, device=dev)
        capi.call("g2pc_pack_geometry", capi.ptr(self.means3D), capi.ptr(self.cov3d), capi.ptr(self.opacity), n,
                  capi.ptr(self._geom), st)
        k = int(config.PREPROCESS_CAMERAS)
        if not 1 <= k <= capi.PREPROCESS_MAX_CAMERAS:
            raise capi.G2pcError(f"config.PREPROCESS_CAMERAS must be 1..{capi.PREPROCESS_MAX_CAMERAS}, got {k}")
        self._init_frames(preprocess_cameras=k)
        self._leaf_colour = None

    def get_gaussians_above_contribution_threshold(self, contribution_threshold):
        self.flush()
        return self.gaussian_max_contribution > contribution_threshold

    def get_visible_gaussians(self):
        return self.get_gaussians_above_contribution_threshold(self.visible_gaussian_threshold)

    def get_surface_gaussians(self):
        self.flush()
        return self.get_gaussians_above_contribution_threshold(torch.mean(self.gaussian_max_contribution))

    def get_total_gaussian_contributions(self):
        self.flush()
        return self.gaussian_max_contribution

    def _get_tables(self, W, H):
        key = (W, H, self.max_tile_size, self.max_gaussians_per_tile, self._extra_levels)
        t = self._tables.get(key)
        if t is None:
            qt = quadtree.QuadtreeTables(W, H, self.max_tile_size, self.max_gaussians_per_tile,
                                         extra_levels=self._extra_levels)
            flat = np.concatenate(qt.flat()).astype(np.int32)
            dev = self.device
            mask = qt.candidate_level_mask()
            base = (mask & -mask).bit_length() - 1
            if base > 8:
                raise capi.G2pcError("image too large for the packed node range (first leaf level deeper than 8)")
            luts = qt.pixel_luts()
            if luts.shape[0] % 2:
                luts = np.concatenate([luts, np.zeros(1, np.uint16)])
            t = dict(qt=qt, tables=torch.from_numpy(flat).to(dev), level_mask=mask, base_level=base,
                     clean_mask=qt.clean_level_mask(),
                     luts=torch.from_numpy(luts.view(np.int16).copy()).to(dev),
                     slots=[dict(node_cnt=torch.zeros((qt.nodes_2d,), dtype=torch.int32, device=dev),
                                 node_state=torch.zeros((qt.nodes_2d,), dtype=torch.uint8, device=dev),
                                 node_leaf=torch.full((qt.nodes_2d,), -1, dtype=torch.int32, device=dev),
                                 leaves=None, leaf_order=None) for _ in range(self.num_slots)],
                     owner=torch.zeros((W * H,), dtype=torch.int32, device=dev),
                     image=torch.ones((H, W, 3), dtype=torch.float32, device=dev),
                     leaf_cap=0, pix_cap=int(1.25 * W * H) + 4096,
                     max_leaf=(int(min(self.max_tile_size, W)), int(min(self.max_tile_size, H))))
            t["pre_cnt"] = [[ts["node_cnt"]] + [torch.zeros((qt.nodes_2d,), dtype=torch.int32, device=dev)
                                                for _ in range(self.preprocess_cameras - 1)] for ts in t["slots"]]
            self._set_leaf_cap(t, min(qt.nodes_2d, 2 * (4 ** base)))
            self._tables[key] = t
        return t

    def _set_leaf_cap(self, t, cap):
        cap = int(min(max(cap, 1), t["qt"].nodes_2d))
        chunk = int(self.lib.g2pc_multisplit_chunk(cap))
        if chunk <= 0:
            raise capi.G2pcError(f"the quadtree has more than {cap} leaves: too many for the multisplit tables")
        t["leaf_cap"], t["chunk"] = cap, chunk
        t["chunks"] = int(self.lib.g2pc_multisplit_rows(self._n, cap))
        for ts in t["slots"]:
            ts["leaves"] = torch.zeros((cap, capi.LEAF_WORDS), dtype=torch.int32, device=self.device)
            ts["leaf_order"] = torch.zeros((cap,), dtype=torch.int32, device=self.device)

    @staticmethod
    def _camera_struct(camera):
        c = capi.Camera()
        if hasattr(camera, "host"):
            get = camera.host
        else:
            get = lambda k: getattr(camera, k).detach().to("cpu", torch.float32)
        V = get("world_view_transform").contiguous().reshape(-1).tolist()
        P = get("projection_matrix").contiguous().reshape(-1).tolist()
        pos = get("camera_center").reshape(-1).tolist()
        for i in range(16):
            c.view[i] = V[i]
            c.proj[i] = P[i]
        for i in range(3):
            c.campos[i] = pos[i]
        c.tan_fovx = math.tan(camera.FoVx * 0.5)
        c.tan_fovy = math.tan(camera.FoVy * 0.5)
        c.focal_x = camera.focal_x
        c.focal_y = camera.focal_y
        c.width = camera.image_width
        c.height = camera.image_height
        return c

    def _ensure_buffers(self, camera, slot):
        t = self._get_tables(int(camera.image_width), int(camera.image_height))
        self._grow_lists(self._slots[slot], t["leaf_cap"], t["chunks"])
        if self._leaf_colour is None or self._leaf_colour.numel() < 3 * t["pix_cap"]:
            self._leaf_colour = torch.empty((3 * t["pix_cap"],), dtype=torch.float32, device=self.device)

    def _enqueue_preprocess(self, cameras, bset):
        st = capi.stream_ptr(self.device)
        k = len(cameras)
        t = self._get_tables(int(cameras[0].image_width), int(cameras[0].image_height))
        qt = t["qt"]
        sets, cnts = self._pre_sets[bset][:k], t["pre_cnt"][bset][:k]
        scene = (capi.ptr(self._geom), capi.ptr(self._colour_f32) if self.shs is None else None, capi.ptr(self.shs),
                 int(self.shs.shape[-1]) if self.shs is not None else 0, self.sh_degree, self._n)
        if k == 1:
            cam = self._camera_struct(cameras[0])
            capi.call("g2pc_preprocess", *scene, ctypes.byref(cam), capi.ptr(t["tables"]), capi.ptr(t["luts"]),
                      qt.num_levels, t["level_mask"], t["clean_mask"], capi.ptr(sets[0]["proj"]), capi.ptr(cnts[0]),
                      capi.ptr(sets[0]["depth_key"]), capi.ptr(sets[0]["val"]), st)
            return
        cams = (capi.Camera * k)(*[self._camera_struct(c) for c in cameras])
        ptrs = lambda ts: (ctypes.c_void_p * k)(*[capi.ptr(x) for x in ts])
        capi.call("g2pc_preprocess_cameras", *scene, cams, k, capi.ptr(t["tables"]), capi.ptr(t["luts"]), qt.num_levels,
                  t["level_mask"], t["clean_mask"], ptrs([x["proj"] for x in sets]), ptrs(cnts),
                  ptrs([x["depth_key"] for x in sets]), ptrs([x["val"] for x in sets]), st)

    def _enqueue_front(self, camera, frame, slot, pre):
        st = capi.stream_ptr(self.device)
        W, H = int(camera.image_width), int(camera.image_height)
        n = self._n
        t = self._get_tables(W, H)
        qt = t["qt"]
        ps, node_cnt = self._pre_sets[pre[0]][pre[1]], t["pre_cnt"][pre[0]][pre[1]]
        sl, ts = self._slots[slot], t["slots"][slot]
        sl["pre"] = ps
        self._depth_sort(sl, st, ps)
        capi.call("g2pc_build_tree", capi.ptr(t["tables"]), qt.num_levels, qt.max_gaussians_per_tile,
                  capi.ptr(node_cnt), capi.ptr(ts["node_state"]), capi.ptr(ts["node_leaf"]), capi.ptr(ts["leaves"]),
                  capi.ptr(ts["leaf_order"]), t["leaf_cap"], self._inst_cap, t["pix_cap"], sl["matrix"].numel(),
                  t["chunks"], frame, capi.ptr(sl["hdr"]), capi.ptr(self._fail), capi.ptr(sl["work"]), st)
        capi.call("g2pc_multisplit", capi.ptr(sl["val_sorted"]), n, capi.ptr(ps["proj"]), W, H, capi.ptr(t["tables"]),
                  qt.num_levels, t["level_mask"], t["clean_mask"], capi.ptr(ts["node_leaf"]), capi.ptr(ts["leaves"]),
                  capi.ptr(sl["hdr"]),
                  capi.ptr(self._fail), frame, t["leaf_cap"], capi.ptr(sl["matrix"]), capi.ptr(sl["inst_gid"]), st)
        self._last_tables, self._last_slot = t, slot
        return sl["hdr"]

    def _enqueue_back(self, camera, frame, camera_index, slot):
        st = capi.stream_ptr(self.device)
        W, H = int(camera.image_width), int(camera.image_height)
        n = self._n
        t = self._get_tables(W, H)
        sl, ts = self._slots[slot], t["slots"][slot]
        bg = 1.0 if self.white_bkgd else 0.0
        capi.call("g2pc_blend", capi.ptr(ts["leaves"]), capi.ptr(ts["leaf_order"]), capi.ptr(sl["hdr"]),
                  capi.ptr(self._fail), frame, *t["max_leaf"], capi.ptr(sl["inst_gid"]), capi.ptr(sl["pre"]["proj"]),
                  capi.ptr(self._cam_best), capi.ptr(self.gaussian_max_contribution), capi.ptr(self._leaf_colour),
                  capi.ptr(t["owner"]), W, H, bg, float(self.t_stop), capi.ptr(sl["work"]), capi.ptr(self._stats), st)
        capi.call("g2pc_accumulate", capi.ptr(self._cam_best), capi.ptr(self._leaf_colour), n,
                  capi.ptr(self.gaussian_max_contribution), capi.ptr(self.gaussian_colours),
                  capi.ptr(self.first_frame), int(camera_index), st)
        if self.compose_image:
            capi.call("g2pc_compose_image", capi.ptr(t["owner"]), capi.ptr(self._leaf_colour), W, H, bg,
                      capi.ptr(t["image"]), st)
        else:
            t["owner"].zero_()

    def __call__(self, camera, camera_index=None, **kwargs):
        self._submit(camera, camera_index)
        if not self.compose_image:
            return None, None, None, None
        if self.async_mode:
            return self._get_tables(int(camera.image_width), int(camera.image_height))["image"], None, None, None
        return self._last_tables["image"].clone(), None, None, None

    def _confirm(self, h):
        t = self._last_tables
        self.last_stats = dict(num_leaves=h[capi.HDR_NUM_LEAVES],
                               total_instances=total_instances(h),
                               total_leaf_pixels=h[capi.HDR_TOTAL_PIX], levels=t["qt"].num_levels, frame=h[capi.HDR_FRAME])

    def _fix(self, h):
        t = self._last_tables
        W, H = t["qt"].width, t["qt"].height
        if h[capi.HDR_NEED_DEEPER]:
            levels = t["qt"].num_levels
            self._extra_levels += 1
            if self._get_tables(W, H)["qt"].num_levels <= levels:
                raise capi.G2pcError(
                    f"a tile still holds more than max_gaussians_per_tile={self.max_gaussians_per_tile} Gaussians at "
                    f"quadtree level {levels - 1} (tiles of a few pixels): deeper than the tabulated levels")
        elif h[capi.HDR_LEAF_OVERFLOW]:
            if t["leaf_cap"] >= t["qt"].nodes_2d:
                raise capi.G2pcError("leaf table overflow")
            self._set_leaf_cap(t, max(2 * t["leaf_cap"], int(1.25 * h[capi.HDR_NUM_LEAVES])))
        elif h[capi.HDR_CAP_OVERFLOW]:
            self._grow_inst_cap(h)
            t["pix_cap"] = max(t["pix_cap"], int(1.25 * h[capi.HDR_TOTAL_PIX]) + 1024)
        else:
            raise capi.G2pcError("poisoned frame header without a cause")

    def debug_last_camera(self):
        self.flush()
        t, sl = self._last_tables, self._slots[self._last_slot]
        nl = self.last_stats["num_leaves"]
        leaves = t["slots"][self._last_slot]["leaves"][:nl].cpu().numpy()
        gids = sl["inst_gid"].cpu().numpy().astype(np.int64) if nl else np.zeros(0, np.int64)
        out = []
        for (r0, c0, w, h, beg, cnt, pix, node) in leaves:
            out.append((int(r0), int(c0), int(w), int(h), gids[beg:beg + cnt]))
        return sl["pre"]["proj"].cpu().numpy(), out


def get_renderer(renderer_type: str, xyz, opacities, colours, covariances, shs=None, visible_gaussian_threshold=0.0,
                 surface_distance_std=None, calculate_surface_distance=False):
    if renderer_type == "python":
        return GaussPythonRenderer(xyz, opacities.type(torch.float), colours if shs is None else None, covariances,
                                   visible_gaussian_threshold=visible_gaussian_threshold, shs=shs)
    if renderer_type == "cuda":
        from g2pc.rasterizer import GaussianRasterizer as GaussianPCRasterizer
        means2D = None
        common = dict(cov3D_precomp=covariances.to(torch.float), visible_gaussian_threshold=visible_gaussian_threshold,
                      surface_distance_std=surface_distance_std, calculate_surface_distance=calculate_surface_distance)
        if shs is None:
            return GaussianPCRasterizer(xyz.to(torch.float), means2D, opacities.type(torch.float),
                                        colors_precomp=colours.to(torch.float), **common)
        return GaussianPCRasterizer(xyz.to(torch.float), means2D, opacities.type(torch.float), shs=shs.to(torch.float),
                                    sh_layout=0, **common)
    raise Exception(f"Renderer of type {renderer_type} is not supported")
```

### include/g2pc.h

```cpp
#ifndef G2PC_H
#define G2PC_H

#include <stdint.h>

#ifdef __cplusplus
extern "C" {
#endif

#define G2PC_OK 0
#define G2PC_ERR_INVALID 1
#define G2PC_ERR_CUDA 2
#define G2PC_ERR_WORKSPACE 3

#define G2PC_F32 0
#define G2PC_F64 1

int g2pc_version(void);
const char* g2pc_last_error(void);

int g2pc_cov_build(const void* scales, const void* rots, int in_dtype, float scale_modifier,
                   int64_t n, float* cov, void* stream);

int g2pc_normals(const void* scales, const void* rots, int in_dtype, int64_t n, float* normals,
                 void* stream);

int g2pc_eigvals_sym3(const float* cov, int64_t n, float* eigvals, void* stream);

typedef struct {
    int32_t j0;
    int32_t count;
    int32_t k;
    int32_t lpg;
} g2pc_tile_t;

typedef struct {
    int32_t attempt;
    int32_t j0;
    int32_t count;
    int32_t k;
} g2pc_unit_t;

#define G2PC_CULL_EPS_NORM 0
#define G2PC_CULL_EXPLICIT 1

#define G2PC_ST_OVERFLOW 0
#define G2PC_ST_CHOLFAIL 1
#define G2PC_ST_CHOLREG 2
#define G2PC_ST_WORDS 4

int g2pc_sample_count(const float* xyz, const float* cov, const void* colours, int colour_dtype,
                      const float* normals, const int32_t* perm, const uint32_t* gids, int64_t gid_offset, int64_t n,
                      const g2pc_tile_t* tiles, int32_t num_tiles, int32_t num_attempts,
                      int32_t attempts_stored, float mahalanobis_std, int32_t cull_mode, uint64_t seed,
                      uint32_t call_id, void* records, uint32_t* xl, uint32_t* tile_totals,
                      int32_t* status, void* stream);

int g2pc_sample_emit_chunk_points(void);
int g2pc_sample_emit(const void* records, const uint32_t* xl, int64_t n, const g2pc_unit_t* units,
                     const int64_t* unit_base, const int32_t* chunk_unit, int32_t num_units, uint64_t seed,
                     uint32_t call_id,
                     float* out_xyz, void* out_rgb, void* out_nrm, int out_dtype, int64_t capacity,
                     void* stream);

int g2pc_dump_eps(const int64_t* gids, int64_t n_gids, int32_t k, int32_t attempt, uint64_t seed,
                  uint32_t call_id, float* eps, void* stream);

int64_t g2pc_cull_workspace_bytes(int64_t n);
int g2pc_cull_select(const float* max_contrib, float vis_threshold, const float* opacity, float min_opacity,
                     const float* xyz, const float* bbox_min3_host, const float* bbox_max3_host,
                     const float* surface_dist, const float* surface_threshold_dev, const uint8_t* extra_mask,
                     int64_t lo, int64_t hi, int64_t n, int32_t* index, int64_t* count, void* workspace,
                     int64_t workspace_bytes, void* stream);
int g2pc_gather_rows(const int32_t* index, int64_t m, int32_t num_arrays, const void* const* srcs, void* const* dsts,
                     const int32_t* row_bytes, void* stream);

int64_t g2pc_ppg_workspace_bytes(int64_t n);
int g2pc_points_per_gaussian(const float* cov, const float* contrib, int64_t n, double num_points, double* magnitudes,
                             int32_t* ppg, void* workspace, int64_t workspace_bytes, void* stream);

#define G2PC_SOR_K_MAX 32

int64_t g2pc_knn_workspace_bytes(int64_t n);
int g2pc_knn_mean_dist(const float* xyz, int64_t n, int32_t k, double* avg, int32_t* status, void* workspace,
                       int64_t workspace_bytes, void* stream);
#define G2PC_ORIENT_K_MAX 31
int g2pc_knn_ids(const float* xyz, int64_t n, int32_t k, int32_t* ids, double* d2, int32_t* status, void* workspace,
                 int64_t workspace_bytes, void* stream);
int64_t g2pc_sor_workspace_bytes(int64_t n);
int g2pc_sor_mask(const double* avg, int64_t n, double std_ratio, uint8_t* keep, double* stats, void* workspace,
                  int64_t workspace_bytes, void* stream);

#define G2PC_MESH_DEPTH_MAX 10
#define G2PC_MESH_FRAME_WORDS 8

int64_t g2pc_mesh_splat_workspace_bytes(int64_t n);
int g2pc_mesh_splat(const float* xyz, const void* normals, int normal_dtype, int64_t n, int32_t depth, double* frame,
                    int64_t* B, uint32_t* cell, int32_t* status, void* workspace, int64_t workspace_bytes, void* stream);

int64_t g2pc_mesh_solve_workspace_bytes(int32_t depth);
int g2pc_mesh_vcycle(const int64_t* B, const double* frame, int32_t depth, float* chi, int32_t first, double* norms,
                     void* workspace, int64_t workspace_bytes, void* stream);

int64_t g2pc_mesh_iso_workspace_bytes(void);
int g2pc_mesh_iso(const float* xyz, const uint32_t* cell, int64_t n, const double* frame, int32_t depth, float* chi,
                  double* iso, void* workspace, int64_t workspace_bytes, void* stream);

int64_t g2pc_mesh_extract_workspace_bytes(int32_t depth);
int g2pc_mesh_extract_count(const float* chi, int32_t depth, const double* iso, int64_t* counts, void* workspace,
                            int64_t workspace_bytes, void* stream);
int g2pc_mesh_extract_emit(const float* chi, int32_t depth, const double* frame, const double* iso, void* node_scratch,
                           int64_t node_scratch_bytes, const void* workspace, int64_t workspace_bytes, int64_t* vkey,
                           double* vt, double* vpos, int32_t* faces, void* stream);

int64_t g2pc_mesh_gather_workspace_bytes(int64_t n);
int g2pc_mesh_gather(const float* xyz, const int32_t* colours, const uint32_t* cell, int64_t n, const double* frame,
                     int32_t depth, const int64_t* vkey, const double* vt, int64_t m, void* cell_scratch,
                     int64_t cell_scratch_bytes, double* density, uint8_t* vcolours, void* workspace,
                     int64_t workspace_bytes, void* stream);

int64_t g2pc_mesh_trim_workspace_bytes(int64_t m, int64_t t);
int g2pc_mesh_trim(const double* density, const double* vpos, const uint8_t* vcolours, int64_t m, const int32_t* faces,
                   int64_t t, uint8_t* keep, double* threshold, int64_t* counts, double* density_out, double* vpos_out,
                   uint8_t* vcolours_out, int32_t* faces_out, void* workspace, int64_t workspace_bytes, void* stream);

int64_t g2pc_mesh_smooth_workspace_bytes(int64_t m, int64_t t);
int g2pc_mesh_smooth(double* vpos, int64_t m, const int32_t* faces, int64_t t, int32_t iterations, void* workspace,
                     int64_t workspace_bytes, void* stream);

int64_t g2pc_mesh_normals_workspace_bytes(int64_t m, int64_t t);
int g2pc_mesh_normals(const double* vpos, int64_t m, const int32_t* faces, int64_t t, float* vertices, float* normals,
                      void* workspace, int64_t workspace_bytes, void* stream);

#define G2PC_MESH_BAND_DEPTH_MAX 12
#define G2PC_MESH_BRICK 8
#define G2PC_MESH_BAND_MARGIN 1
#define G2PC_MESH_CG_WORDS 5

int64_t g2pc_mesh_band_bricks_workspace_bytes(int32_t depth);
int g2pc_mesh_band_bricks(const float* xyz, const uint32_t* cell, int64_t n, const double* frame, int32_t depth,
                          const int32_t* parent_map, double* band_frame, int32_t* map, int64_t* counts, void* workspace,
                          int64_t workspace_bytes, void* stream);
int g2pc_mesh_band_list(const int32_t* map, int32_t depth, int32_t* list, void* stream);
int g2pc_mesh_band_splat(const float* xyz, const void* normals, int normal_dtype, const uint32_t* cell, int64_t n,
                         const double* band_frame, int32_t depth, const int32_t* map, int64_t nbricks, int64_t* B,
                         int32_t* status, void* stream);
int g2pc_mesh_band_ghosts(const float* parent_chi, const int32_t* parent_map, int32_t depth, const int32_t* map,
                          const int32_t* list, int64_t nbricks, const int64_t* B, const double* band_frame,
                          double* ghost, float* chi, float* rhs, void* stream);
int64_t g2pc_mesh_band_cg_workspace_bytes(int64_t nbricks);
int g2pc_mesh_band_cg_start(const float* rhs, int32_t depth, const int32_t* map, const int32_t* list, int64_t nbricks,
                            float* chi, double* scalars, void* workspace, int64_t workspace_bytes, void* stream);
int g2pc_mesh_band_cg_step(const float* rhs, int32_t depth, const int32_t* map, const int32_t* list, int64_t nbricks,
                           float* chi, int32_t iteration, double* scalars, void* workspace, int64_t workspace_bytes,
                           void* stream);
int64_t g2pc_mesh_band_iso_workspace_bytes(void);
int g2pc_mesh_band_iso(const float* xyz, const uint32_t* cell, int64_t n, const double* band_frame, int32_t depth,
                       const int32_t* map, const float* chi, double* iso, void* workspace, int64_t workspace_bytes,
                       void* stream);
int64_t g2pc_mesh_band_extract_workspace_bytes(int64_t nbricks);
int g2pc_mesh_band_extract_count(const float* chi, int32_t depth, const int32_t* map, const int32_t* list,
                                 int64_t nbricks, const double* iso, int64_t* counts, void* workspace,
                                 int64_t workspace_bytes, void* stream);
int g2pc_mesh_band_extract_emit(const float* chi, int32_t depth, const int32_t* map, const int32_t* list,
                                int64_t nbricks, const double* band_frame, const double* iso, void* node_scratch,
                                int64_t node_scratch_bytes, const void* workspace, int64_t workspace_bytes,
                                int64_t* vkey, double* vt, double* vpos, int32_t* faces, void* stream);
int64_t g2pc_mesh_band_gather_workspace_bytes(int64_t n);
int g2pc_mesh_band_gather(const float* xyz, const int32_t* colours, const uint32_t* cell, int64_t n,
                          const double* band_frame, int32_t depth, const int64_t* vkey, const double* vt, int64_t m,
                          double* density, uint8_t* vcolours, void* workspace, int64_t workspace_bytes, void* stream);

int64_t g2pc_mesh_decimate_prepare_workspace_bytes(int64_t m, int64_t t);
int g2pc_mesh_decimate_prepare(const double* vpos, int64_t m, const int32_t* faces, int64_t t, double* quadrics,
                               uint8_t* free_flags, void* workspace, int64_t workspace_bytes, void* stream);
int64_t g2pc_mesh_decimate_round_workspace_bytes(int64_t m, int64_t t);
int g2pc_mesh_decimate_select(const double* vpos, int64_t m, const int32_t* faces, int64_t t, const double* quadrics,
                              const uint8_t* free_flags, int64_t* counts, void* workspace, int64_t workspace_bytes,
                              void* stream);
int g2pc_mesh_decimate_apply(double* vpos, int64_t m, const int32_t* faces, int64_t t, double* quadrics,
                             int64_t* colour_sums, int32_t* merged, double* density_sums, uint8_t* alive,
                             int64_t selected, int64_t k, int32_t* faces_out, int64_t* kept, uint64_t* applied,
                             int32_t* applied_ab, void* workspace, int64_t workspace_bytes, void* stream);
int64_t g2pc_mesh_decimate_finish_workspace_bytes(int64_t m);
int g2pc_mesh_decimate_finish(const double* vpos, int64_t m, const int32_t* faces, int64_t t, const uint8_t* alive,
                              const int64_t* colour_sums, const int32_t* merged, const double* density_sums,
                              double* vpos_out, uint8_t* colours_out, double* densities_out, int32_t* faces_out,
                              int64_t* counts, void* workspace, int64_t workspace_bytes, void* stream);


int64_t g2pc_orient_prepare_workspace_bytes(int64_t n);
int g2pc_orient_prepare(const float* xyz, const void* normals, int normal_dtype, int64_t n, int32_t* rows, float* uxyz,
                        double* unh, int64_t* count, void* workspace, int64_t workspace_bytes, void* stream);

int64_t g2pc_orient_edges_workspace_bytes(int64_t m, int32_t k);
int g2pc_orient_edges(const int32_t* ids, int64_t m, int32_t k, const double* unh, uint64_t* edges, uint64_t* keys,
                      uint8_t* flips, int64_t* count, void* workspace, int64_t workspace_bytes, void* stream);

int64_t g2pc_orient_round_workspace_bytes(int64_t m, int64_t c);
int g2pc_orient_round(const uint64_t* edges, const uint64_t* keys, const uint8_t* flips, int64_t m, int64_t c,
                      int32_t round_index, int64_t active, int32_t* comp, uint8_t* rel, uint8_t* mst, int64_t* counts,
                      void* workspace, int64_t workspace_bytes, void* stream);

int64_t g2pc_orient_finish_workspace_bytes(int64_t m);
int g2pc_orient_finish(const float* uxyz, const double* unh, const int32_t* rows, int64_t m, const void* normals,
                       int normal_dtype, int64_t n, const int32_t* comp, const uint8_t* rel, void* out, int32_t* seed,
                       uint8_t* seed_rel, int64_t* stats, void* workspace, int64_t workspace_bytes, void* stream);

int g2pc_face_cameras(const float* means, const void* normals, int normal_dtype, const int32_t* ids, int64_t m,
                      const int32_t* cam_of, int64_t n, const float* cams, int64_t ncam, void* out, int64_t* counts,
                      void* stream);

typedef struct {
    float view[16];
    float proj[16];
    float campos[3];
    float tan_fovx, tan_fovy, focal_x, focal_y;
    int32_t width, height;
} g2pc_camera_t;

typedef struct {
    int32_t r0, c0, w, h;
    int32_t inst_begin;
    int32_t inst_count;
    int32_t pix_offset;
    int32_t node;
} g2pc_leaf_t;

#define G2PC_MAX_LEVELS 12
#define G2PC_HDR_NUM_LEAVES 0
#define G2PC_HDR_TOTAL_INST 1
#define G2PC_HDR_TOTAL_PIX 2
#define G2PC_HDR_NEED_DEEPER 3
#define G2PC_HDR_LEAF_OVERFLOW 4
#define G2PC_HDR_CAP_OVERFLOW 5
#define G2PC_HDR_POISON 6
#define G2PC_HDR_FRAME 7
#define G2PC_HDR_TOTAL_INST_HI 8
#define G2PC_HDR_WORDS 16
#define G2PC_WORK_COUNTERS 4
#define G2PC_STAT_WARP_GAUSSIANS 0
#define G2PC_STAT_WORDS 4



int g2pc_pack_geometry(const float* xyz, const float* cov, const float* opacity, int64_t n, void* geom, void* stream);

int g2pc_preprocess(const void* geom, const float* colours, const float* shs, int32_t sh_stride, int32_t sh_degree,
                    int64_t n, const g2pc_camera_t* cam_host, const int32_t* tables, const uint16_t* luts,
                    int32_t num_levels, uint32_t level_mask, uint32_t clean_mask, void* proj, uint32_t* node_cnt,
                    uint32_t* depth_key, uint64_t* val, void* stream);

#define G2PC_PREPROCESS_MAX_CAMERAS 8
int g2pc_preprocess_cameras(const void* geom, const float* colours, const float* shs, int32_t sh_stride,
                            int32_t sh_degree, int64_t n, const g2pc_camera_t* cams_host, int32_t num_cameras,
                            const int32_t* tables, const uint16_t* luts, int32_t num_levels, uint32_t level_mask,
                            uint32_t clean_mask, void* const* proj, uint32_t* const* node_cnt,
                            uint32_t* const* depth_key, uint64_t* const* val, void* stream);

int64_t g2pc_depth_sort_workspace_bytes(int64_t n);
int g2pc_depth_sort(const uint32_t* depth_key, const uint64_t* val, int64_t n, uint64_t* val_sorted, void* workspace,
                    int64_t workspace_bytes, void* stream);

int g2pc_build_tree(const int32_t* tables, int32_t num_levels, int32_t max_gaussians_per_tile, uint32_t* node_cnt,
                    uint8_t* node_state, int32_t* node_leaf, g2pc_leaf_t* leaves, int32_t* leaf_order,
                    int32_t max_leaves, int64_t inst_capacity, int64_t pix_capacity, int64_t matrix_capacity,
                    int32_t ms_chunks, int32_t frame, int32_t* header, uint32_t* fail, int32_t* work_counters,
                    void* stream);

int32_t g2pc_multisplit_chunk(int32_t leaf_cap);
int32_t g2pc_multisplit_rows(int64_t n, int32_t leaf_cap);
int g2pc_multisplit(const uint64_t* val_sorted, int64_t n, const void* proj, int32_t width, int32_t height,
                    const int32_t* tables, int32_t num_levels, uint32_t level_mask, uint32_t clean_mask,
                    const int32_t* node_leaf, const g2pc_leaf_t* leaves, const int32_t* header, const uint32_t* fail,
                    int32_t frame,
                    int32_t leaf_cap, uint32_t* matrix, uint32_t* inst_gid, void* stream);

int g2pc_blend(const g2pc_leaf_t* leaves, const int32_t* leaf_order, const int32_t* header, const uint32_t* fail,
               int32_t frame, int32_t max_leaf_width, int32_t max_leaf_height, const uint32_t* inst_gid, const void* proj,
               uint64_t* cam_best,
               const float* max_contrib, float* leaf_colour, uint32_t* owner, int32_t width, int32_t height,
               float background, float t_stop, int32_t* work_counters, uint64_t* stats, void* stream);

void g2pc_blend_set_compact(int on);

void g2pc_blend_set_cull(int on);

int g2pc_accumulate(uint64_t* cam_best, const float* leaf_colour, int64_t n, float* max_contrib, float* colours,
                    int32_t* first_frame, int32_t frame, void* stream);

int g2pc_compose_image(uint32_t* owner, const float* leaf_colour, int32_t width, int32_t height, float background,
                       float* image, void* stream);

typedef struct {
    float viewmatrix[16];
    float projmatrix[16];
    float campos[3];
    float tan_fovx, tan_fovy;
    int32_t width, height;
} g2pc_raster_t;

int g2pc_tiles_preprocess(const void* geom, const float* colours, const float* shs, int32_t sh_stride,
                          int32_t sh_degree, int32_t sh_layout, int64_t n, const g2pc_raster_t* rs_host, void* proj,
                          uint32_t* node_cnt, uint32_t* depth_key, uint64_t* val, int32_t* radii, void* stream);

int g2pc_tiles_build(uint32_t* node_cnt, int32_t width, int32_t height, g2pc_leaf_t* leaves, int32_t* leaf_order,
                     int32_t max_leaves, int64_t inst_capacity, int64_t matrix_capacity, int32_t ms_rows, int32_t frame,
                     int32_t* header, uint32_t* fail, int32_t* work_counters, void* stream);

int g2pc_multisplit_grid(const uint64_t* val_sorted, int64_t n, int32_t grid_w, int32_t grid_h,
                         const g2pc_leaf_t* leaves, const int32_t* header, const uint32_t* fail, int32_t frame,
                         int32_t leaf_cap, uint32_t* matrix, uint32_t* inst_gid, void* stream);

int g2pc_tiles_blend(const g2pc_leaf_t* leaves, const int32_t* leaf_order, const int32_t* header, const uint32_t* fail,
                     int32_t frame, const uint32_t* inst_gid, const void* proj, uint64_t* cam_best, uint32_t* cam_dist,
                     const int32_t* mask, float* out_color, float* out_depth, float* out_invdepth, int32_t width,
                     int32_t height, const float* background3_host, int32_t* work_counters, uint64_t* stats,
                     void* stream);

int g2pc_tiles_blend_fusion(const g2pc_leaf_t* leaves, const int32_t* leaf_order, const int32_t* header,
                            const uint32_t* fail, int32_t frame, const uint32_t* inst_gid, const void* proj,
                            uint64_t* cam_best, uint32_t* cam_dist, const int32_t* mask, float* out_color,
                            float* out_depth, float* out_invdepth, int32_t width, int32_t height,
                            const float* background3_host, int32_t* work_counters, uint64_t* stats, float* out_T,
                            float* out_zmed, void* stream);

int g2pc_tiles_accumulate(uint64_t* cam_best, uint32_t* cam_dist, const float* out_color, int32_t width, int32_t height,
                          int64_t n, float* max_contrib, float* total_contrib, float* colours, float* min_dist,
                          int32_t* first_frame, int32_t frame, float* cam_contrib, int32_t* cam_pixel,
                          float* cam_surface, void* stream);

int g2pc_fill_u32(uint32_t* v, uint32_t value, int64_t n, void* stream);

int64_t g2pc_tsdf_frame_workspace_bytes(int64_t n);
int g2pc_tsdf_frame(const float* xyz, int64_t n, int32_t depth, double* frame, void* workspace, int64_t workspace_bytes,
                    void* stream);

int g2pc_tsdf_integrate(const double* frame, int32_t depth, double trunc_voxels, const float* zmed,
                        const float* transmittance, const float* image, const int32_t* mask, int32_t width,
                        int32_t height, const g2pc_raster_t* rs_host, const float* background3_host,
                        const uint32_t* fail, int32_t frame_index, float* tsdf, float* weight, float* colour,
                        void* stream);

int64_t g2pc_tsdf_compact_workspace_bytes(int64_t m, int64_t t);
int g2pc_tsdf_gather_compact(const float* weight, const float* colour, int32_t depth, const int64_t* vkey,
                             const double* vt, const double* vpos, int64_t m, const int32_t* faces, int64_t t,
                             uint8_t* keep, double* density, uint8_t* vcolours, int64_t* counts, double* density_out,
                             double* vpos_out, uint8_t* vcolours_out, int32_t* faces_out, void* workspace,
                             int64_t workspace_bytes, void* stream);

#ifdef __cplusplus
}
#endif
#endif
```

Before: 32.33.

## Replace matrix multisplit with two-level row/column split of sorted instances

Replaces the leaf-count matrix multisplit for the base grid with a two-pass split: instances are first bucketed by grid row using warp bit-transposes and per-band counts, then each row list is split by column into inst_gid, with shared-memory staging for coalesced writes. The old matrix multisplit kernels now only run when a base cell needs deeper quadtree levels, gated by a device-side base_split flag. The aim is to cut the cost of the per-leaf histogram matrix and its scan. In exchange it needs a row-list workspace with its own capacity and overflow handling, and images are limited to 256 super-tiles per axis.

```diff
diff --git a/3dgs-to-pc_b200/csrc/colour_common.cuh b/3dgs-to-pc_b200/csrc/colour_common.cuh
--- a/3dgs-to-pc_b200/csrc/colour_common.cuh
+++ b/3dgs-to-pc_b200/csrc/colour_common.cuh
@@ -39,6 +39,7 @@
     header[G2PC_HDR_LEAF_OVERFLOW] = leaf_over;
     header[G2PC_HDR_CAP_OVERFLOW] = cap_over;
     header[G2PC_HDR_FRAME] = frame;
+    header[G2PC_HDR_ROW_INST] = 0;
     if (need_deeper | leaf_over | cap_over) atomicMin(fail, (uint32_t)(frame + 1));
     const uint32_t f = *(volatile uint32_t*)fail;
     header[G2PC_HDR_POISON] = f == 0xFFFFFFFFu ? 0 : (int32_t)f;
diff --git a/3dgs-to-pc_b200/csrc/core.cu b/3dgs-to-pc_b200/csrc/core.cu
--- a/3dgs-to-pc_b200/csrc/core.cu
+++ b/3dgs-to-pc_b200/csrc/core.cu
@@ -10,5 +10,5 @@
     va_end(ap);
 }
 
-extern "C" int g2pc_version(void) { return 110; }
+extern "C" int g2pc_version(void) { return 111; }
 extern "C" const char* g2pc_last_error(void) { return g_err; }
diff --git a/3dgs-to-pc_b200/csrc/s4_tree.cu b/3dgs-to-pc_b200/csrc/s4_tree.cu
--- a/3dgs-to-pc_b200/csrc/s4_tree.cu
+++ b/3dgs-to-pc_b200/csrc/s4_tree.cu
@@ -158,35 +158,26 @@
     int32_t leaf_cap;
     int32_t base_clean;
     uint32_t clean_mask;
-    int32_t grid_w;
+    const uint32_t* base_split;
     int32_t steps;
 };
 
 template <typename F>
 __device__ __forceinline__ void for_each_leaf(const MsParams& p, const QtTables& T, const int32_t* __restrict__ s_leaf,
                                               uint32_t range, uint32_t gid, F f) {
-    if (p.grid_w > 0) {
-        warp_for_each_node(range, gid, [&](int ix, int iy, int owner, uint32_t og) { f(iy * p.grid_w + ix, owner, og); });
-        return;
-    }
     const int lb = p.base_level;
     const int o1 = (1 << lb) - 1;
     unsigned deeper = 0;
     if (p.base_clean) {
-        warp_for_each_node(range, gid, [&](int ix, int iy, int owner, uint32_t og) {
-            const int32_t v = s_leaf[(iy << lb) + ix];
-            if (v >= 0) f(v, owner, og);
-            else if (v == -2) deeper |= 1u << owner;
+        warp_for_each_node(range, gid, [&](int ix, int iy, int owner, uint32_t) {
+            if (s_leaf[(iy << lb) + ix] == -2) deeper |= 1u << owner;
         });
     } else {
-        warp_for_each_node(range, gid, [&](int ix, int iy, int owner, uint32_t og) {
+        warp_for_each_node(range, gid, [&](int ix, int iy, int owner, uint32_t) {
             if (!axis_member(T.ys + o1, T.ye + o1, T.yf + o1, iy) || !axis_member(T.xs + o1, T.xe + o1, T.xf + o1, ix)) return;
-            const int32_t v = s_leaf[(iy << lb) + ix];
-            if (v >= 0) f(v, owner, og);
-            else if (v == -2) deeper |= 1u << owner;
+            if (s_leaf[(iy << lb) + ix] == -2) deeper |= 1u << owner;
         });
     }
-    if (p.meta.num_levels <= lb + 1) return;
     int xlo, xhi, ylo, yhi;
     g2pc_unpack_range(range, xlo, xhi, ylo, yhi);
 #pragma unroll
@@ -242,13 +233,7 @@
 }
 
 __device__ __forceinline__ int32_t* ms_load_common(const MsParams& p, int32_t* smem, QtTables& T) {
-    if (p.grid_w > 0) { T = p.tab; return smem; }
-    if (p.base_clean && p.meta.num_levels <= p.base_level + 1) {
-        T = p.tab;
-        __syncthreads();
-    } else {
-        T = load_tables(p.tab, p.n1, smem);
-    }
+    T = load_tables(p.tab, p.n1, smem);
     int32_t* s_leaf = smem + 6 * p.n1;
     const int nb = 1 << (2 * p.base_level);
     const int32_t* src = p.node_leaf + off2d(p.base_level);
@@ -259,11 +244,11 @@
 template <int C>
 __global__ void __launch_bounds__(C, 1024 / C) ms_count_kernel(const MsParams p) {
     extern __shared__ int32_t smem_ms[];
-    if (g2pc_frame_skipped(p.fail, p.frame)) return;
+    if (g2pc_frame_skipped(p.fail, p.frame) || *p.base_split == 0u) return;
     const int nl = p.header[G2PC_HDR_NUM_LEAVES];
     QtTables T;
     int32_t* s_leaf = ms_load_common(p, smem_ms, T);
-    uint32_t* s_hist = reinterpret_cast<uint32_t*>(s_leaf + (p.grid_w > 0 ? 0 : (1 << (2 * p.base_level))));
+    uint32_t* s_hist = reinterpret_cast<uint32_t*>(s_leaf + (1 << (2 * p.base_level)));
     for (int i = threadIdx.x; i < nl; i += C) s_hist[i] = 0u;
     __syncthreads();
     const int64_t k0 = (int64_t)blockIdx.x * p.steps * C;
@@ -282,7 +267,7 @@
 constexpr int SCAN_BATCH = 8;
 __global__ void __launch_bounds__(1024) ms_scan_kernel(const MsParams p, int32_t rows) {
     __shared__ uint32_t s_sum[32][33];
-    if (g2pc_frame_skipped(p.fail, p.frame)) return;
+    if (g2pc_frame_skipped(p.fail, p.frame) || *p.base_split == 0u) return;
     const int nl = p.header[G2PC_HDR_NUM_LEAVES];
     if (blockIdx.x * 32 >= nl) return;
     const int tx = threadIdx.x & 31, ty = threadIdx.x >> 5;
@@ -315,12 +300,12 @@
 template <int C>
 __global__ void __launch_bounds__(C, 768 / C) ms_scatter_kernel(const MsParams p) {
     extern __shared__ int32_t smem_ms[];
-    if (g2pc_frame_skipped(p.fail, p.frame)) return;
+    if (g2pc_frame_skipped(p.fail, p.frame) || *p.base_split == 0u) return;
     const int nl = p.header[G2PC_HDR_NUM_LEAVES];
     constexpr int WORDS = C / 32;
     QtTables T;
     int32_t* s_leaf = ms_load_common(p, smem_ms, T);
-    uint32_t* s_row = reinterpret_cast<uint32_t*>(s_leaf + (p.grid_w > 0 ? 0 : (1 << (2 * p.base_level))));
+    uint32_t* s_row = reinterpret_cast<uint32_t*>(s_leaf + (1 << (2 * p.base_level)));
     uint32_t* s_bits = s_row + p.leaf_cap;
     {
         const uint32_t* grow = p.matrix + (int64_t)blockIdx.x * nl;
@@ -366,7 +351,394 @@
     }
 }
 
+constexpr int SP_BATCHES = 8;
+constexpr int SP_TILE = 32 * SP_BATCHES;
+constexpr int SP_WARPS = 16;
+constexpr int SP_BAND = SP_TILE * SP_WARPS;
+constexpr int SP_MAX_CELLS = 256;
+constexpr int SP_MAX_GROUPS = SP_MAX_CELLS / 32;
+constexpr int SP_STAGE_BYTES = 6 * 1024;
+
+struct SplitParams {
+    const unsigned long long* val_sorted;
+    int64_t n;
+    int32_t rows, cols;
+    int32_t rows_p, cols_p;
+    const int32_t* cell_leaf;
+    QtTables tab;
+    int32_t clean;
+    const g2pc_leaf_t* leaves;
+    int32_t* header;
+    uint32_t* fail;
+    int32_t frame;
+    unsigned long long* row_list;
+    int64_t row_capacity;
+    uint32_t* m1;
+    uint32_t* b1;
+    uint32_t* m2;
+    uint32_t* b2;
+    uint32_t* row_begin;
+    uint32_t* band_begin;
+    uint32_t* base_split;
+    int32_t bands1;
+    uint32_t* inst_gid;
+};
+
+__device__ __forceinline__ uint32_t span_bits(int lo, int hi, int base) {
+    lo = max(lo - base, 0);
+    hi = min(hi - base, 31);
+    return lo > hi ? 0u : ((0xFFFFFFFFu >> (31 - hi)) & (0xFFFFFFFFu << lo));
+}
+
+__device__ __forceinline__ uint32_t warp_transpose32(uint32_t x) {
+    const int lane = threadIdx.x & 31;
+    const uint32_t masks[5] = {0x0000FFFFu, 0x00FF00FFu, 0x0F0F0F0Fu, 0x33333333u, 0x55555555u};
+#pragma unroll
+    for (int i = 0, s = 16; i < 5; ++i, s >>= 1) {
+        const uint32_t t = __shfl_xor_sync(0xffffffffu, x, s);
+        x = (lane & s) ? ((x & ~masks[i]) | ((t & ~masks[i]) >> s)) : ((x & masks[i]) | ((t & masks[i]) << s));
+    }
+    return x;
+}
+
+template <int LEVEL, int G, bool COUNT, typename Out>
+__device__ __forceinline__ void split_walk(const SplitParams& p, const unsigned long long* __restrict__ src, int64_t beg,
+                                           int64_t end, const uint32_t (&member)[G], uint32_t (&acc)[G], Out out) {
+    const int lane = threadIdx.x & 31;
+    for (int64_t b = beg; b < end; b += 32) {
+        const int64_t k = b + lane;
+        const unsigned long long v = k < end ? src[k] : (unsigned long long)G2PC_RANGE_EMPTY << 32;
+        int xlo, xhi, ylo, yhi;
+        g2pc_unpack_range((uint32_t)(v >> 32), xlo, xhi, ylo, yhi);
+        const bool some = xlo <= xhi && ylo <= yhi;
+        const int lo = LEVEL == 1 ? ylo : xlo, hi = LEVEL == 1 ? yhi : xhi;
+#pragma unroll
+        for (int g = 0; g < G; ++g) {
+            const uint32_t m = some ? span_bits(lo, hi, 32 * g) & member[g] : 0u;
+            if (G > 1 && !__any_sync(0xffffffffu, m != 0u)) continue;
+            const uint32_t bal = warp_transpose32(m);
+            if (COUNT) {
+                acc[g] += (uint32_t)__popc(bal);
+                continue;
+            }
+            uint32_t rem = bal, pos = acc[g];
+            while (__any_sync(0xffffffffu, rem != 0u)) {
+                const int s = rem ? __ffs(rem) - 1 : 0;
+                if (LEVEL == 1) {
+                    const uint32_t lo32 = __shfl_sync(0xffffffffu, (uint32_t)v, s);
+                    const uint32_t hi32 = __shfl_sync(0xffffffffu, (uint32_t)(v >> 32), s);
+                    if (rem) out(pos++, ((unsigned long long)hi32 << 32) | lo32);
+                } else {
+                    const uint32_t gid = __shfl_sync(0xffffffffu, (uint32_t)v, s);
+                    if (rem) out(pos++, (unsigned long long)gid);
+                }
+                rem &= rem - 1u;
+            }
+            acc[g] = pos;
+        }
+    }
+}
+
+template <int LEVEL, int G>
+__device__ __forceinline__ void split_members(const SplitParams& p, int row, uint32_t (&member)[G]) {
+    const int lane = threadIdx.x & 31;
+#pragma unroll
+    for (int g = 0; g < G; ++g) {
+        const int c = 32 * g + lane;
+        bool in;
+        if (LEVEL == 1) {
+            in = c < p.rows && (p.clean || axis_member(p.tab.ys, p.tab.ye, p.tab.yf, c));
+        } else {
+            in = c < p.cols && (p.cell_leaf == nullptr || p.cell_leaf[row * p.cols + c] >= 0) &&
+                 (p.clean || axis_member(p.tab.xs, p.tab.xe, p.tab.xf, c));
+        }
+        member[g] = __ballot_sync(0xffffffffu, in);
+    }
+}
+
+__device__ __forceinline__ int split_band_row(const SplitParams& p, int band, int64_t& beg, int64_t& end) {
+    int lo = 0, hi = p.rows - 1;
+    while (lo < hi) {
+        const int mid = (lo + hi + 1) >> 1;
+        if ((int)p.band_begin[mid] <= band) lo = mid; else hi = mid - 1;
+    }
+    beg = (int64_t)p.row_begin[lo] + (int64_t)(band - (int)p.band_begin[lo]) * SP_BAND;
+    end = min(beg + SP_BAND, (int64_t)p.row_begin[lo + 1]);
+    return lo;
+}
+
+template <int LEVEL, int G>
+__global__ void __launch_bounds__(32 * SP_WARPS) split_count_kernel(const SplitParams p) {
+    __shared__ uint32_t s_cnt[SP_WARPS][32 * G];
+    if (g2pc_frame_skipped(p.fail, p.frame)) return;
+    const int lane = threadIdx.x & 31, w = threadIdx.x >> 5, band = blockIdx.x;
+    int64_t beg, end;
+    int row = 0;
+    if (LEVEL == 1) {
+        beg = (int64_t)band * SP_BAND;
+        end = min(beg + SP_BAND, p.n);
+    } else {
+        if (band >= (int)p.band_begin[p.rows]) return;
+        row = split_band_row(p, band, beg, end);
+    }
+    uint32_t member[G], cnt[G];
+    split_members<LEVEL, G>(p, row, member);
+#pragma unroll
+    for (int g = 0; g < G; ++g) cnt[g] = 0u;
+    const int64_t tb = beg + (int64_t)w * SP_TILE;
+    split_walk<LEVEL, G, true>(p, LEVEL == 1 ? p.val_sorted : p.row_list, tb, min(tb + SP_TILE, end), member, cnt,
+                               [](uint32_t, unsigned long long) {});
+#pragma unroll
+    for (int g = 0; g < G; ++g) s_cnt[w][32 * g + lane] = cnt[g];
+    __syncthreads();
+    const int width = 32 * G;
+    uint32_t* m = (LEVEL == 1 ? p.m1 : p.m2) + (int64_t)band * (SP_WARPS + 1) * width;
+    for (int c = threadIdx.x; c < width; c += 32 * SP_WARPS) {
+        uint32_t run = 0;
+#pragma unroll
+        for (int w2 = 0; w2 < SP_WARPS; ++w2) {
+            m[w2 * width + c] = run;
+            run += s_cnt[w2][c];
+        }
+        m[SP_WARPS * width + c] = run;
+        (LEVEL == 1 ? p.b1 : p.b2)[(int64_t)band * width + c] = run;
+    }
+}
+
+template <int LEVEL, int G>
+__global__ void __launch_bounds__(32 * SP_WARPS) split_scatter_kernel(const SplitParams p) {
+    using T = typename std::conditional<LEVEL == 1, unsigned long long, uint32_t>::type;
+    extern __shared__ __align__(16) unsigned char smem_sp[];
+    if (g2pc_frame_skipped(p.fail, p.frame)) return;
+    const int lane = threadIdx.x & 31, w = threadIdx.x >> 5, band = blockIdx.x;
+    int64_t beg, end;
+    int row = 0;
+    if (LEVEL == 1) {
+        beg = (int64_t)band * SP_BAND;
+        end = min(beg + SP_BAND, p.n);
+    } else {
+        if (band >= (int)p.band_begin[p.rows]) return;
+        row = split_band_row(p, band, beg, end);
+    }
+    const int64_t tb = beg + (int64_t)w * SP_TILE;
+    if (tb >= end) return;
+    const int width = 32 * G;
+    const uint32_t* m = (LEVEL == 1 ? p.m1 : p.m2) + ((int64_t)band * (SP_WARPS + 1) + w) * width;
+    const uint32_t* bo = (LEVEL == 1 ? p.b1 : p.b2) + (int64_t)band * width;
+    T* dst = LEVEL == 1 ? (T*)p.row_list : (T*)p.inst_gid;
+    uint32_t member[G], off[G], cnt[G], sbeg[G], pos[G];
+    split_members<LEVEL, G>(p, row, member);
+    uint32_t total = 0;
+#pragma unroll
+    for (int g = 0; g < G; ++g) {
+        const uint32_t m0 = m[32 * g + lane];
+        off[g] = bo[32 * g + lane] + m0;
+        cnt[g] = m[width + 32 * g + lane] - m0;
+        uint32_t inc = cnt[g];
+#pragma unroll
+        for (int o = 1; o < 32; o <<= 1) {
+            const uint32_t t = __shfl_up_sync(0xffffffffu, inc, o);
+            if (lane >= o) inc += t;
+        }
+        sbeg[g] = total + inc - cnt[g];
+        total += __shfl_sync(0xffffffffu, inc, 31);
+    }
+    const int64_t te = min(tb + SP_TILE, end);
+    constexpr int CAP = SP_STAGE_BYTES / (int)sizeof(T);
+    if (total > (uint32_t)CAP) {
+        split_walk<LEVEL, G, false>(p, LEVEL == 1 ? p.val_sorted : p.row_list, tb, te, member, off,
+                                    [&](uint32_t q, unsigned long long x) { dst[q] = (T)x; });
+        return;
+    }
+    T* stage = reinterpret_cast<T*>(smem_sp + w * SP_STAGE_BYTES);
+#pragma unroll
+    for (int g = 0; g < G; ++g) pos[g] = sbeg[g];
+    split_walk<LEVEL, G, false>(p, LEVEL == 1 ? p.val_sorted : p.row_list, tb, te, member, pos,
+                                [&](uint32_t q, unsigned long long x) { stage[q] = (T)x; });
+    __syncwarp();
+#pragma unroll
+    for (int g = 0; g < G; ++g) {
+        unsigned todo = __ballot_sync(0xffffffffu, cnt[g] != 0u);
+        while (todo) {
+            const int b = __ffs(todo) - 1;
+            todo &= todo - 1u;
+            const uint32_t len = __shfl_sync(0xffffffffu, cnt[g], b), s0 = __shfl_sync(0xffffffffu, sbeg[g], b);
+            const uint32_t d0 = __shfl_sync(0xffffffffu, off[g], b);
+            for (uint32_t k = lane; k < len; k += 32) dst[d0 + k] = stage[s0 + k];
+        }
+    }
+}
+
+__global__ void __launch_bounds__(1024) split_rows_scan_kernel(const SplitParams p) {
+    __shared__ uint32_t s_part[SP_MAX_GROUPS][32][33];
+    __shared__ uint32_t s_begin[SP_MAX_CELLS];
+    __shared__ int s_over;
+    if (g2pc_frame_skipped(p.fail, p.frame)) return;
+    if (p.base_split) {
+        int split = 0;
+        for (int i = threadIdx.x; i < p.rows * p.cols; i += 1024) split |= p.cell_leaf[i] == -2;
+        split = __syncthreads_or(split);
+        if (threadIdx.x == 0) *p.base_split = split ? 1u : 0u;
+    }
+    const int tx = threadIdx.x & 31, ty = threadIdx.x >> 5;
+    const int groups = p.rows_p / 32;
+    const int per = (p.bands1 + 31) / 32;
+    const int c0 = min(p.bands1, ty * per), c1 = min(p.bands1, c0 + per);
+    for (int g = 0; g < groups; ++g) {
+        const uint32_t* col = p.b1 + 32 * g + tx;
+        uint32_t sum = 0;
+#pragma unroll 8
+        for (int c = c0; c < c1; ++c) sum += col[(int64_t)c * p.rows_p];
+        s_part[g][ty][tx] = sum;
+    }
+    __syncthreads();
+    if (ty == 0) {
+        unsigned long long tot[SP_MAX_GROUPS], bands[SP_MAX_GROUPS], st = 0, sb = 0;
+#pragma unroll
+        for (int i = 0; i < SP_MAX_GROUPS; ++i) {
+            const int r = tx * SP_MAX_GROUPS + i;
+            uint32_t t = 0;
+            if (r < p.rows)
+                for (int s = 0; s < 32; ++s) t += s_part[r >> 5][s][r & 31];
+            tot[i] = t;
+            bands[i] = (t + SP_BAND - 1) / SP_BAND;
+            st += tot[i];
+            sb += bands[i];
+        }
+        unsigned long long it = st, ib = sb;
+#pragma unroll
+        for (int o = 1; o < 32; o <<= 1) {
+            const unsigned long long a = __shfl_up_sync(0xffffffffu, it, o), b = __shfl_up_sync(0xffffffffu, ib, o);
+            if (tx >= o) { it += a; ib += b; }
+        }
+        unsigned long long rt = it - st, rb = ib - sb;
+        const unsigned long long total = __shfl_sync(0xffffffffu, it, 31);
+        const bool over = total > (unsigned long long)p.row_capacity;
+        if (!over) {
+#pragma unroll
+            for (int i = 0; i < SP_MAX_GROUPS; ++i) {
+                const int r = tx * SP_MAX_GROUPS + i;
+                if (r < p.rows) {
+                    p.row_begin[r] = (uint32_t)rt;
+                    p.band_begin[r] = (uint32_t)rb;
+                    s_begin[r] = (uint32_t)rt;
+                }
+                rt += tot[i];
+                rb += bands[i];
+            }
+            if (tx == 31) {
+                p.row_begin[p.rows] = (uint32_t)rt;
+                p.band_begin[p.rows] = (uint32_t)rb;
+            }
+        }
+        if (tx == 0) {
+            s_over = over ? 1 : 0;
+            p.header[G2PC_HDR_ROW_INST] = (int32_t)min(total, 0x7FFFFFFFull);
+            if (over) {
+                p.header[G2PC_HDR_CAP_OVERFLOW] = 1;
+                atomicMin(p.fail, (uint32_t)(p.frame + 1));
+                p.header[G2PC_HDR_POISON] = (int32_t)*(volatile uint32_t*)p.fail;
+            }
+        }
+    }
+    __syncthreads();
+    if (s_over) return;
+    for (int g = 0; g < groups; ++g) {
+        const int r = 32 * g + tx;
+        if (r >= p.rows) continue;
+        uint32_t run = s_begin[r];
+        for (int s = 0; s < ty; ++s) run += s_part[g][s][tx];
+        uint32_t* col = p.b1 + r;
+        for (int c = c0; c < c1; ++c) {
+            const uint32_t t = col[(int64_t)c * p.rows_p];
+            col[(int64_t)c * p.rows_p] = run;
+            run += t;
+        }
+    }
+}
+
+__global__ void __launch_bounds__(256) split_cols_scan_kernel(const SplitParams p) {
+    if (g2pc_frame_skipped(p.fail, p.frame)) return;
+    const int i = blockIdx.x * 256 + threadIdx.x;
+    const int row = i / p.cols_p, c = i - row * p.cols_p;
+    if (row >= p.rows) return;
+    uint32_t run = 0;
+    if (c < p.cols) {
+        const int leaf = p.cell_leaf ? p.cell_leaf[row * p.cols + c] : row * p.cols + c;
+        if (leaf >= 0) run = (uint32_t)p.leaves[leaf].inst_begin;
+    }
+    const int b0 = (int)p.band_begin[row], b1 = (int)p.band_begin[row + 1];
+    uint32_t* col = p.b2 + c;
+    for (int b = b0; b < b1; ++b) {
+        const uint32_t t = col[(int64_t)b * p.cols_p];
+        col[(int64_t)b * p.cols_p] = run;
+        run += t;
+    }
+}
+
 size_t align256(size_t x) { return (x + 255) & ~(size_t)255; }
+
+int64_t split_bands1(int64_t n) { return (n + SP_BAND - 1) / SP_BAND; }
+int64_t split_bands2(int64_t row_capacity, int rows) { return (row_capacity + SP_BAND - 1) / SP_BAND + rows; }
+
+int64_t split_workspace_bytes(int64_t n, int64_t row_capacity, int rows, int cols) {
+    const int64_t rp = (rows + 31) / 32 * 32, cp = (cols + 31) / 32 * 32;
+    const int64_t b1 = split_bands1(n), b2 = split_bands2(row_capacity, rows);
+    return (int64_t)(align256(4) + align256((size_t)row_capacity * 8) + align256((size_t)(b1 * (SP_WARPS + 1) * rp * 4)) +
+                     align256((size_t)(b1 * rp * 4)) + align256((size_t)(b2 * (SP_WARPS + 1) * cp * 4)) +
+                     align256((size_t)(b2 * cp * 4)) + 2 * align256((size_t)(rows + 1) * 4));
+}
+
+template <int LEVEL, int G>
+void split_launch_level(const SplitParams& p, int64_t bands, cudaStream_t st) {
+    split_count_kernel<LEVEL, G><<<(unsigned)bands, 32 * SP_WARPS, 0, st>>>(p);
+    if (LEVEL == 1) split_rows_scan_kernel<<<1, 1024, 0, st>>>(p);
+    else split_cols_scan_kernel<<<(unsigned)((p.rows * p.cols_p + 255) / 256), 256, 0, st>>>(p);
+    constexpr size_t smem = (size_t)SP_WARPS * SP_STAGE_BYTES;
+    cudaFuncSetAttribute(split_scatter_kernel<LEVEL, G>, cudaFuncAttributeMaxDynamicSharedMemorySize, (int)smem);
+    split_scatter_kernel<LEVEL, G><<<(unsigned)bands, 32 * SP_WARPS, smem, st>>>(p);
+}
+
+template <int LEVEL>
+void split_level(const SplitParams& p, int64_t bands, cudaStream_t st) {
+    switch ((LEVEL == 1 ? p.rows_p : p.cols_p) / 32) {
+        case 1: split_launch_level<LEVEL, 1>(p, bands, st); break;
+        case 2: split_launch_level<LEVEL, 2>(p, bands, st); break;
+        case 3: split_launch_level<LEVEL, 3>(p, bands, st); break;
+        case 4: split_launch_level<LEVEL, 4>(p, bands, st); break;
+        case 5: split_launch_level<LEVEL, 5>(p, bands, st); break;
+        case 6: split_launch_level<LEVEL, 6>(p, bands, st); break;
+        case 7: split_launch_level<LEVEL, 7>(p, bands, st); break;
+        default: split_launch_level<LEVEL, 8>(p, bands, st); break;
+    }
+}
+
+int run_split(SplitParams p, void* workspace, int64_t workspace_bytes, cudaStream_t st) {
+    if (workspace_bytes < split_workspace_bytes(p.n, p.row_capacity, p.rows, p.cols)) {
+        g2pc_set_error("g2pc_multisplit: workspace smaller than g2pc_multisplit_workspace_bytes");
+        return G2PC_ERR_WORKSPACE;
+    }
+    p.rows_p = (p.rows + 31) / 32 * 32;
+    p.cols_p = (p.cols + 31) / 32 * 32;
+    const int64_t b1 = split_bands1(p.n), b2 = split_bands2(p.row_capacity, p.rows);
+    char* ws = (char*)workspace;
+    auto take = [&](size_t bytes) { char* q = ws; ws += align256(bytes); return q; };
+    uint32_t* flag = (uint32_t*)take(4);
+    p.base_split = p.cell_leaf ? flag : nullptr;
+    p.row_list = (unsigned long long*)take((size_t)p.row_capacity * 8);
+    p.m1 = (uint32_t*)take((size_t)(b1 * (SP_WARPS + 1) * p.rows_p * 4));
+    p.b1 = (uint32_t*)take((size_t)(b1 * p.rows_p * 4));
+    p.m2 = (uint32_t*)take((size_t)(b2 * (SP_WARPS + 1) * p.cols_p * 4));
+    p.b2 = (uint32_t*)take((size_t)(b2 * p.cols_p * 4));
+    p.row_begin = (uint32_t*)take((size_t)(p.rows + 1) * 4);
+    p.band_begin = (uint32_t*)take((size_t)(p.rows + 1) * 4);
+    p.bands1 = (int32_t)b1;
+    split_level<1>(p, b1, st);
+    split_level<2>(p, b2, st);
+    G2PC_CHECK_LAUNCH();
+    return G2PC_OK;
+}
+
 
 constexpr int64_t MS_TARGET_CTAS = 4096;
 constexpr int64_t MS_MAX_STEPS = 32;
@@ -382,7 +754,7 @@
 
 template <int C>
 int launch_multisplit(const MsParams& p, int32_t chunks, cudaStream_t st) {
-    const size_t common = p.grid_w > 0 ? 0 : ((size_t)6 * p.n1 + ((size_t)1 << (2 * p.base_level))) * sizeof(int32_t);
+    const size_t common = ((size_t)6 * p.n1 + ((size_t)1 << (2 * p.base_level))) * sizeof(int32_t);
     const size_t smem_count = common + (size_t)p.leaf_cap * sizeof(uint32_t);
     const size_t smem_scatter = common + (size_t)(C / 32 + 1) * p.leaf_cap * sizeof(uint32_t);
     if (smem_scatter > 200 * 1024 || smem_count > 200 * 1024) {
@@ -474,51 +846,73 @@
     return ms_chunks(n, C);
 }
 
+extern "C" int64_t g2pc_multisplit_workspace_bytes(int64_t n, int64_t row_capacity, int32_t grid_w, int32_t grid_h) {
+    if (n < 0 || row_capacity < 0 || grid_w < 1 || grid_h < 1 || grid_w > SP_MAX_CELLS || grid_h > SP_MAX_CELLS) return -1;
+    return split_workspace_bytes(n, row_capacity, grid_h, grid_w);
+}
+
 extern "C" int g2pc_multisplit(const uint64_t* val_sorted, int64_t n, const void* proj, int32_t width, int32_t height,
                                const int32_t* tables, int32_t num_levels, uint32_t level_mask, uint32_t clean_mask,
-                               const int32_t* node_leaf,
-                               const g2pc_leaf_t* leaves, const int32_t* header, const uint32_t* fail, int32_t frame,
-                               int32_t leaf_cap, uint32_t* matrix, uint32_t* inst_gid, void* stream) {
+                               const int32_t* node_leaf, const g2pc_leaf_t* leaves, int32_t* header,
+                               const uint32_t* fail, int32_t frame, int32_t leaf_cap, uint32_t* matrix,
+                               int64_t row_capacity, void* workspace, int64_t workspace_bytes, uint32_t* inst_gid,
+                               void* stream) {
     G2PC_CHECK_ARG(n >= 0, "n < 0");
     if (n == 0) return G2PC_OK;
-    G2PC_CHECK_ARG(val_sorted && proj && tables && node_leaf && leaves && header && fail && matrix && inst_gid,
+    G2PC_CHECK_ARG(val_sorted && proj && tables && node_leaf && leaves && header && fail && workspace && inst_gid,
                    "null pointer");
     G2PC_CHECK_ARG(num_levels >= 1 && num_levels <= G2PC_MAX_LEVELS && level_mask != 0u, "bad levels");
+    G2PC_CHECK_ARG(row_capacity >= 0 && row_capacity <= 0x7FFFFFFFll, "bad row capacity");
+    const int base = __builtin_ctz(level_mask);
+    G2PC_CHECK_ARG(base <= G2PC_RANGE_MAX_LEVEL, "first leaf-candidate level too deep");
+    const int n1 = (1 << num_levels) - 1, o1 = (1 << base) - 1;
+    const QtTables tab = make_tables(tables, n1);
+    cudaStream_t st = (cudaStream_t)stream;
+    SplitParams s{};
+    s.val_sorted = (const unsigned long long*)val_sorted; s.n = n;
+    s.rows = s.cols = 1 << base;
+    s.cell_leaf = node_leaf + off2d(base);
+    s.tab.xs = tab.xs + o1; s.tab.xe = tab.xe + o1; s.tab.xf = tab.xf + o1;
+    s.tab.ys = tab.ys + o1; s.tab.ye = tab.ye + o1; s.tab.yf = tab.yf + o1;
+    s.clean = (int32_t)((clean_mask >> base) & 1u);
+    s.leaves = leaves; s.header = header; s.fail = const_cast<uint32_t*>(fail); s.frame = frame;
+    s.row_capacity = row_capacity; s.inst_gid = inst_gid;
+    const int rc = run_split(s, workspace, workspace_bytes, st);
+    if (rc != G2PC_OK || num_levels <= base + 1) return rc;
     const int C = g2pc_multisplit_chunk(leaf_cap);
     G2PC_CHECK_ARG(C > 0, "too many leaves for the multisplit");
+    G2PC_CHECK_ARG(matrix, "null matrix with levels below the base level");
     MsParams p;
     p.val_sorted = (const unsigned long long*)val_sorted; p.n = n; p.proj = (const float4*)proj;
     p.width = width; p.height = height;
     p.inv_width = 1.0f / (float)width; p.inv_height = 1.0f / (float)height;
     p.meta.num_levels = num_levels; p.meta.max_gaussians_per_tile = 0; p.meta.width = width; p.meta.height = height;
-    p.n1 = (1 << num_levels) - 1;
-    p.tab = make_tables(tables, p.n1);
-    p.level_mask = level_mask; p.base_level = __builtin_ctz(level_mask);
-    G2PC_CHECK_ARG(p.base_level <= G2PC_RANGE_MAX_LEVEL, "first leaf-candidate level too deep");
+    p.n1 = n1;
+    p.tab = tab;
+    p.level_mask = level_mask; p.base_level = base;
     p.node_leaf = node_leaf; p.header = header; p.fail = fail; p.frame = frame; p.leaves = leaves; p.matrix = matrix;
     p.inst_gid = inst_gid;
-    p.leaf_cap = leaf_cap; p.grid_w = 0;
-    p.base_clean = (int32_t)((clean_mask >> p.base_level) & 1u);
+    p.leaf_cap = leaf_cap;
+    p.base_clean = s.clean;
     p.clean_mask = clean_mask;
-    return run_multisplit(p, C, (cudaStream_t)stream);
+    p.base_split = (const uint32_t*)workspace;
+    return run_multisplit(p, C, st);
 }
 
 extern "C" int g2pc_multisplit_grid(const uint64_t* val_sorted, int64_t n, int32_t grid_w, int32_t grid_h,
-                                    const g2pc_leaf_t* leaves, const int32_t* header, const uint32_t* fail,
-                                    int32_t frame, int32_t leaf_cap, uint32_t* matrix, uint32_t* inst_gid, void* stream) {
+                                    const g2pc_leaf_t* leaves, int32_t* header, const uint32_t* fail, int32_t frame,
+                                    int64_t row_capacity, void* workspace, int64_t workspace_bytes, uint32_t* inst_gid,
+                                    void* stream) {
     G2PC_CHECK_ARG(n >= 0, "n < 0");
     if (n == 0) return G2PC_OK;
-    G2PC_CHECK_ARG(val_sorted && leaves && header && fail && matrix && inst_gid, "null pointer");
-    G2PC_CHECK_ARG(grid_w >= 1 && grid_h >= 1 && grid_w <= 256 && grid_h <= 256 && leaf_cap >= grid_w * grid_h,
-                   "bad tile grid / leaf_cap");
-    const int C = g2pc_multisplit_chunk(leaf_cap);
-    G2PC_CHECK_ARG(C > 0, "too many tiles for the multisplit");
-    MsParams p{};
-    p.val_sorted = (const unsigned long long*)val_sorted; p.n = n;
-    p.meta.num_levels = 1;
-    p.level_mask = 1u;
-    p.header = header; p.fail = fail; p.frame = frame; p.leaves = leaves; p.matrix = matrix;
-    p.inst_gid = inst_gid;
-    p.leaf_cap = leaf_cap; p.grid_w = grid_w; p.base_clean = 1; p.clean_mask = 1u;
-    return run_multisplit(p, C, (cudaStream_t)stream);
-}
+    G2PC_CHECK_ARG(val_sorted && leaves && header && fail && workspace && inst_gid, "null pointer");
+    G2PC_CHECK_ARG(grid_w >= 1 && grid_h >= 1 && grid_w <= SP_MAX_CELLS && grid_h <= SP_MAX_CELLS, "bad tile grid");
+    G2PC_CHECK_ARG(row_capacity >= 0 && row_capacity <= 0x7FFFFFFFll, "bad row capacity");
+    SplitParams s{};
+    s.val_sorted = (const unsigned long long*)val_sorted; s.n = n;
+    s.rows = grid_h; s.cols = grid_w;
+    s.clean = 1;
+    s.leaves = leaves; s.header = header; s.fail = const_cast<uint32_t*>(fail); s.frame = frame;
+    s.row_capacity = row_capacity; s.inst_gid = inst_gid;
+    return run_split(s, workspace, workspace_bytes, (cudaStream_t)stream);
+}
diff --git a/3dgs-to-pc_b200/g2pc/capi.py b/3dgs-to-pc_b200/g2pc/capi.py
--- a/3dgs-to-pc_b200/g2pc/capi.py
+++ b/3dgs-to-pc_b200/g2pc/capi.py
@@ -136,8 +136,10 @@
                          _i64, _i32, _i32, _c_void_p, _c_void_p, _c_void_p, _c_void_p], ctypes.c_int),
     "g2pc_multisplit_chunk": ([_i32], ctypes.c_int32),
     "g2pc_multisplit_rows": ([_i64, _i32], ctypes.c_int32),
+    "g2pc_multisplit_workspace_bytes": ([_i64, _i64, _i32, _i32], ctypes.c_int64),
     "g2pc_multisplit": ([_c_void_p, _i64, _c_void_p, _i32, _i32, _c_void_p, _i32, _u32, _u32, _c_void_p, _c_void_p,
-                         _c_void_p, _c_void_p, _i32, _i32, _c_void_p, _c_void_p, _c_void_p], ctypes.c_int),
+                         _c_void_p, _c_void_p, _i32, _i32, _c_void_p, _i64, _c_void_p, _i64, _c_void_p, _c_void_p],
+                        ctypes.c_int),
     "g2pc_blend": ([_c_void_p, _c_void_p, _c_void_p, _c_void_p, _i32, _i32, _i32, _c_void_p, _c_void_p, _c_void_p,
                     _c_void_p, _c_void_p, _c_void_p, _i32, _i32, _f32, _f32, _c_void_p, _c_void_p, _c_void_p],
                    ctypes.c_int),
@@ -148,7 +150,7 @@
                                _c_void_p, _c_void_p, _c_void_p, _c_void_p], ctypes.c_int),
     "g2pc_tiles_build": ([_c_void_p, _i32, _i32, _c_void_p, _c_void_p, _i32, _i64, _i64, _i32, _i32, _c_void_p,
                           _c_void_p, _c_void_p, _c_void_p], ctypes.c_int),
-    "g2pc_multisplit_grid": ([_c_void_p, _i64, _i32, _i32, _c_void_p, _c_void_p, _c_void_p, _i32, _i32, _c_void_p,
+    "g2pc_multisplit_grid": ([_c_void_p, _i64, _i32, _i32, _c_void_p, _c_void_p, _c_void_p, _i32, _i64, _c_void_p, _i64,
                               _c_void_p, _c_void_p], ctypes.c_int),
     "g2pc_tiles_blend": ([_c_void_p, _c_void_p, _c_void_p, _c_void_p, _i32, _c_void_p, _c_void_p, _c_void_p, _c_void_p,
                           _c_void_p, _c_void_p, _c_void_p, _c_void_p, _i32, _i32, _c_void_p, _c_void_p, _c_void_p,
@@ -174,7 +176,7 @@
 
 
 (HDR_NUM_LEAVES, HDR_TOTAL_INST, HDR_TOTAL_PIX, HDR_NEED_DEEPER, HDR_LEAF_OVERFLOW, HDR_CAP_OVERFLOW, HDR_POISON,
- HDR_FRAME, HDR_TOTAL_INST_HI) = range(9)
+ HDR_FRAME, HDR_TOTAL_INST_HI, HDR_ROW_INST) = range(10)
 HDR_WORDS = 16
 WORK_COUNTERS = 4
 STAT_WARP_GAUSSIANS, STAT_WORDS = 0, 4
@@ -208,7 +210,7 @@
 
 LAUNCHES = 0
 TIMING = None
-_OWN_KERNELS = {"g2pc_multisplit": 3, "g2pc_multisplit_grid": 3, "g2pc_depth_sort": 0, "g2pc_cull_select": 3,
+_OWN_KERNELS = {"g2pc_multisplit": 6, "g2pc_multisplit_grid": 6, "g2pc_depth_sort": 0, "g2pc_cull_select": 3,
                 "g2pc_points_per_gaussian": 5, "g2pc_knn_mean_dist": 6, "g2pc_knn_ids": 6, "g2pc_sor_mask": 5, "g2pc_mesh_splat": 5,
                 "g2pc_mesh_iso": 7, "g2pc_mesh_extract_count": 2, "g2pc_mesh_extract_emit": 2, "g2pc_mesh_gather": 3,
                 "g2pc_mesh_trim": 6, "g2pc_mesh_normals": 3, "g2pc_mesh_band_bricks": 4, "g2pc_mesh_band_cg_start": 4,
diff --git a/3dgs-to-pc_b200/g2pc/frames.py b/3dgs-to-pc_b200/g2pc/frames.py
--- a/3dgs-to-pc_b200/g2pc/frames.py
+++ b/3dgs-to-pc_b200/g2pc/frames.py
@@ -38,24 +38,28 @@
                             depth_ws=torch.empty((max(nbytes, 1),), dtype=torch.uint8, device=dev),
                             hdr=torch.zeros((capi.HDR_WORDS,), dtype=torch.int32, device=dev),
                             work=torch.zeros((capi.WORK_COUNTERS,), dtype=torch.int32, device=dev),
-                            inst_gid=None, matrix=None) for _ in range(self.num_slots)]
+                            inst_gid=None, matrix=None, ms_ws=None) for _ in range(self.num_slots)]
         self._pre_sets = [[sl] + [None] * (preprocess_cameras - 1) for sl in self._slots]
         self._set_free = [None] * self.num_slots
         self._pre_stream = torch.cuda.Stream(device=self.device) if preprocess_cameras > 1 else None
         self._cam_best = torch.zeros((m,), dtype=torch.int64, device=dev)
         self._stats = torch.zeros((capi.STAT_WORDS,), dtype=torch.int64, device=dev)
         self._inst_cap = max(8 * self._n, 1 << 16)
+        self._row_cap = max(4 * self._n, 1 << 16)
         self._tables = {}
         self._last_slot = 0
         self.last_stats = {}
 
-    def _grow_lists(self, sl, leaf_cap, rows):
+    def _grow_lists(self, sl, leaf_cap, rows, grid):
         need = self._inst_cap + 4 * leaf_cap + 64
         if sl["inst_gid"] is None or sl["inst_gid"].numel() < need:
             sl["inst_gid"] = torch.empty((need,), dtype=torch.int32, device=self.device)
         mneed = rows * leaf_cap
-        if sl["matrix"] is None or sl["matrix"].numel() < mneed:
-            sl["matrix"] = torch.empty((max(mneed, 1),), dtype=torch.int32, device=self.device)
+        if mneed > 0 and (sl["matrix"] is None or sl["matrix"].numel() < mneed):
+            sl["matrix"] = torch.empty((mneed,), dtype=torch.int32, device=self.device)
+        wneed = int(self.lib.g2pc_multisplit_workspace_bytes(max(self._n, 1), self._row_cap, *grid))
+        if sl["ms_ws"] is None or sl["ms_ws"].numel() < wneed:
+            sl["ms_ws"] = capi.workspace(wneed, self.device)
 
     def _depth_sort(self, sl, stream, pre=None):
         pre = sl if pre is None else pre
@@ -67,6 +71,12 @@
         if total > 0x7FFFFFFF:
             raise capi.G2pcError(f"{total} (Gaussian, tile) instances in one camera: more than 2^31 - 1")
         self._inst_cap = max(self._inst_cap, int(1.25 * total) + 1024)
+
+    def _grow_row_cap(self, h):
+        need = h[capi.HDR_ROW_INST]
+        if need >= 0x7FFFFFFF:
+            raise capi.G2pcError("2^31 - 1 or more row-list entries in one camera")
+        self._row_cap = max(self._row_cap, min(int(1.25 * need) + 1024, 0x7FFFFFFF))
 
     def _reset_counts(self):
         for t in self._tables.values():
diff --git a/3dgs-to-pc_b200/g2pc/rasterizer.py b/3dgs-to-pc_b200/g2pc/rasterizer.py
--- a/3dgs-to-pc_b200/g2pc/rasterizer.py
+++ b/3dgs-to-pc_b200/g2pc/rasterizer.py
@@ -141,10 +141,9 @@
             dev = self.device
             gx, gy = ((W + TILE - 1) // TILE + 1) // 2, ((H + TILE - 1) // TILE + 1) // 2
             ntiles = gx * gy
-            chunk = int(self.lib.g2pc_multisplit_chunk(ntiles))
-            if chunk <= 0:
-                raise capi.G2pcError(f"{ntiles} tiles: image too large for the multisplit tables")
-            t = dict(gx=gx, gy=gy, ntiles=ntiles, rows=int(self.lib.g2pc_multisplit_rows(self._n, ntiles)),
+            if gx > 256 or gy > 256:
+                raise capi.G2pcError(f"{gx} x {gy} super-tiles: image too large for the multisplit (256 per axis)")
+            t = dict(gx=gx, gy=gy, ntiles=ntiles,
                      slots=[dict(node_cnt=torch.zeros((ntiles,), dtype=torch.int32, device=dev),
                                  leaves=torch.zeros((ntiles, capi.LEAF_WORDS), dtype=torch.int32, device=dev),
                                  leaf_order=torch.zeros((ntiles,), dtype=torch.int32, device=dev))
@@ -168,7 +167,7 @@
     def _ensure_buffers(self, rs, slot):
         self._pack(float(rs.scale_modifier))
         t = self._res_tables(int(rs.image_width), int(rs.image_height))
-        self._grow_lists(self._slots[slot], t["ntiles"], t["rows"])
+        self._grow_lists(self._slots[slot], t["ntiles"], 0, (t["gx"], t["gy"]))
         self._slots[slot]["mask"] = self._mask_of(rs, int(rs.image_width), int(rs.image_height))
 
     def _enqueue_front(self, rs, frame, slot, pre=None):
@@ -185,11 +184,11 @@
                   capi.ptr(sl["radii"]), st)
         self._depth_sort(sl, st)
         capi.call("g2pc_tiles_build", capi.ptr(ts["node_cnt"]), W, H, capi.ptr(ts["leaves"]), capi.ptr(ts["leaf_order"]),
-                  t["ntiles"], self._inst_cap, sl["matrix"].numel(), t["rows"], frame, capi.ptr(sl["hdr"]),
+                  t["ntiles"], self._inst_cap, 0, 0, frame, capi.ptr(sl["hdr"]),
                   capi.ptr(self._fail), capi.ptr(sl["work"]), st)
         capi.call("g2pc_multisplit_grid", capi.ptr(sl["val_sorted"]), n, t["gx"], t["gy"], capi.ptr(ts["leaves"]),
-                  capi.ptr(sl["hdr"]), capi.ptr(self._fail), frame, t["ntiles"], capi.ptr(sl["matrix"]),
-                  capi.ptr(sl["inst_gid"]), st)
+                  capi.ptr(sl["hdr"]), capi.ptr(self._fail), frame, self._row_cap, capi.ptr(sl["ms_ws"]),
+                  sl["ms_ws"].numel(), capi.ptr(sl["inst_gid"]), st)
         self._last, self._last_slot = t, slot
         return sl["hdr"]
 
@@ -228,6 +227,7 @@
         if not h[capi.HDR_CAP_OVERFLOW]:
             raise capi.G2pcError("failed frame header without a recoverable cause")
         self._grow_inst_cap(h)
+        self._grow_row_cap(h)
 
     def update_max_contributions(self, new_gauss_contributions, new_gauss_colours):
         self.flush()
diff --git a/3dgs-to-pc_b200/gauss_render.py b/3dgs-to-pc_b200/gauss_render.py
--- a/3dgs-to-pc_b200/gauss_render.py
+++ b/3dgs-to-pc_b200/gauss_render.py
@@ -122,7 +122,8 @@
         if chunk <= 0:
             raise capi.G2pcError(f"the quadtree has more than {cap} leaves: too many for the multisplit tables")
         t["leaf_cap"], t["chunk"] = cap, chunk
-        t["chunks"] = int(self.lib.g2pc_multisplit_rows(self._n, cap))
+        deeper = t["qt"].num_levels > t["base_level"] + 1
+        t["chunks"] = int(self.lib.g2pc_multisplit_rows(self._n, cap)) if deeper else 0
         for ts in t["slots"]:
             ts["leaves"] = torch.zeros((cap, capi.LEAF_WORDS), dtype=torch.int32, device=self.device)
             ts["leaf_order"] = torch.zeros((cap,), dtype=torch.int32, device=self.device)
@@ -152,7 +153,7 @@
 
     def _ensure_buffers(self, camera, slot):
         t = self._get_tables(int(camera.image_width), int(camera.image_height))
-        self._grow_lists(self._slots[slot], t["leaf_cap"], t["chunks"])
+        self._grow_lists(self._slots[slot], t["leaf_cap"], t["chunks"], (1 << max(t["base_level"], 0),) * 2)
         if self._leaf_colour is None or self._leaf_colour.numel() < 3 * t["pix_cap"]:
             self._leaf_colour = torch.empty((3 * t["pix_cap"],), dtype=torch.float32, device=self.device)
 
@@ -188,12 +189,14 @@
         self._depth_sort(sl, st, ps)
         capi.call("g2pc_build_tree", capi.ptr(t["tables"]), qt.num_levels, qt.max_gaussians_per_tile,
                   capi.ptr(node_cnt), capi.ptr(ts["node_state"]), capi.ptr(ts["node_leaf"]), capi.ptr(ts["leaves"]),
-                  capi.ptr(ts["leaf_order"]), t["leaf_cap"], self._inst_cap, t["pix_cap"], sl["matrix"].numel(),
+                  capi.ptr(ts["leaf_order"]), t["leaf_cap"], self._inst_cap, t["pix_cap"],
+                  sl["matrix"].numel() if t["chunks"] else 0,
                   t["chunks"], frame, capi.ptr(sl["hdr"]), capi.ptr(self._fail), capi.ptr(sl["work"]), st)
         capi.call("g2pc_multisplit", capi.ptr(sl["val_sorted"]), n, capi.ptr(ps["proj"]), W, H, capi.ptr(t["tables"]),
                   qt.num_levels, t["level_mask"], t["clean_mask"], capi.ptr(ts["node_leaf"]), capi.ptr(ts["leaves"]),
                   capi.ptr(sl["hdr"]),
-                  capi.ptr(self._fail), frame, t["leaf_cap"], capi.ptr(sl["matrix"]), capi.ptr(sl["inst_gid"]), st)
+                  capi.ptr(self._fail), frame, t["leaf_cap"], capi.ptr(sl["matrix"]) if t["chunks"] else None,
+                  self._row_cap, capi.ptr(sl["ms_ws"]), sl["ms_ws"].numel(), capi.ptr(sl["inst_gid"]), st)
         self._last_tables, self._last_slot = t, slot
         return sl["hdr"]
 
@@ -247,6 +250,7 @@
             self._set_leaf_cap(t, max(2 * t["leaf_cap"], int(1.25 * h[capi.HDR_NUM_LEAVES])))
         elif h[capi.HDR_CAP_OVERFLOW]:
             self._grow_inst_cap(h)
+            self._grow_row_cap(h)
             t["pix_cap"] = max(t["pix_cap"], int(1.25 * h[capi.HDR_TOTAL_PIX]) + 1024)
         else:
             raise capi.G2pcError("poisoned frame header without a cause")
diff --git a/include/g2pc.h b/include/g2pc.h
--- a/include/g2pc.h
+++ b/include/g2pc.h
@@ -236,6 +236,7 @@
 #define G2PC_HDR_POISON 6
 #define G2PC_HDR_FRAME 7
 #define G2PC_HDR_TOTAL_INST_HI 8
+#define G2PC_HDR_ROW_INST 9
 #define G2PC_HDR_WORDS 16
 #define G2PC_WORK_COUNTERS 4
 #define G2PC_STAT_WARP_GAUSSIANS 0
@@ -269,11 +270,12 @@
 
 int32_t g2pc_multisplit_chunk(int32_t leaf_cap);
 int32_t g2pc_multisplit_rows(int64_t n, int32_t leaf_cap);
+int64_t g2pc_multisplit_workspace_bytes(int64_t n, int64_t row_capacity, int32_t grid_w, int32_t grid_h);
 int g2pc_multisplit(const uint64_t* val_sorted, int64_t n, const void* proj, int32_t width, int32_t height,
                     const int32_t* tables, int32_t num_levels, uint32_t level_mask, uint32_t clean_mask,
-                    const int32_t* node_leaf, const g2pc_leaf_t* leaves, const int32_t* header, const uint32_t* fail,
-                    int32_t frame,
-                    int32_t leaf_cap, uint32_t* matrix, uint32_t* inst_gid, void* stream);
+                    const int32_t* node_leaf, const g2pc_leaf_t* leaves, int32_t* header, const uint32_t* fail,
+                    int32_t frame, int32_t leaf_cap, uint32_t* matrix, int64_t row_capacity, void* workspace,
+                    int64_t workspace_bytes, uint32_t* inst_gid, void* stream);
 
 int g2pc_blend(const g2pc_leaf_t* leaves, const int32_t* leaf_order, const int32_t* header, const uint32_t* fail,
                int32_t frame, int32_t max_leaf_width, int32_t max_leaf_height, const uint32_t* inst_gid, const void* proj,
@@ -308,8 +310,9 @@
                      int32_t* header, uint32_t* fail, int32_t* work_counters, void* stream);
 
 int g2pc_multisplit_grid(const uint64_t* val_sorted, int64_t n, int32_t grid_w, int32_t grid_h,
-                         const g2pc_leaf_t* leaves, const int32_t* header, const uint32_t* fail, int32_t frame,
-                         int32_t leaf_cap, uint32_t* matrix, uint32_t* inst_gid, void* stream);
+                         const g2pc_leaf_t* leaves, int32_t* header, const uint32_t* fail, int32_t frame,
+                         int64_t row_capacity, void* workspace, int64_t workspace_bytes, uint32_t* inst_gid,
+                         void* stream);
 
 int g2pc_tiles_blend(const g2pc_leaf_t* leaves, const int32_t* leaf_order, const int32_t* header, const uint32_t* fail,
                      int32_t frame, const uint32_t* inst_gid, const void* proj, uint64_t* cam_best, uint32_t* cam_dist,
```

Result: faster. 37.16 (median of 6 runs) (+14.9%).
